# JeroendenBoef/GraphPOPE

Hardware: NVIDIA B200
Metric: anchor-BFS GTEPS (K*|E|/s), geodesic GraphPOPE embedding, Flickr-shape K=256 per GPU (higher is better)
Workload: dtype u64

## Files before the change

graphpope_b200/csrc/gp_api.cu:

```cuda
#include "gp_msbfs.cuh"

#include <algorithm>
#include <atomic>
#include <condition_variable>
#include <functional>
#include <mutex>
#if defined(__x86_64__) || defined(_M_X64)
#include <emmintrin.h>
#endif
#include <thread>
#include <vector>

#include <nvtx3/nvToolsExt.h>
#include <unistd.h>

bool gp_is_capturing();
bool gp_xcopy_tma_ok(const float *d_x, int64_t num_features, int64_t ld_x, const float *d_out, int64_t ld_out);
int gp_launch_xcopy_tma(const float *d_x, int64_t num_nodes, int64_t num_features, int64_t ld_x, float *d_out,
                        int64_t ld_out, cudaStream_t stream);
struct gp_exchange;
int gp_exchange_launch(gp_exchange *x, int parity, const float *d_x, int64_t f, int64_t ldx, float *d_out, int64_t ldo,
                       int64_t coff, cudaStream_t stream);
int gp_exchange_next_parity(gp_exchange *x);
static bool g_capturing_flag_for_count() { return gp_is_capturing(); }
void gp_count_launches(int n);

namespace {
thread_local char g_err[512] = "";
int g_sm_count = 0;
std::atomic<long long> g_launches{0};
}

static thread_local int g_capture_count = 0;
void gp_count_launch()
{
    if (g_capturing_flag_for_count()) ++g_capture_count;
    else g_launches.fetch_add(1, std::memory_order_relaxed);
}
void gp_count_launches(int n) { g_launches.fetch_add(n, std::memory_order_relaxed); }

extern "C" int64_t gp_launch_count(void) { return (int64_t)g_launches.load(); }

void gp_set_error(const char *fmt, ...)
{
    va_list ap;
    va_start(ap, fmt);
    vsnprintf(g_err, sizeof(g_err), fmt, ap);
    va_end(ap);
}

int gp_sm_count()
{
    if (g_sm_count == 0) {
        int dev = 0, sms = 0;
        if (cudaGetDevice(&dev) == cudaSuccess &&
            cudaDeviceGetAttribute(&sms, cudaDevAttrMultiProcessorCount, dev) == cudaSuccess && sms > 0)
            g_sm_count = sms;
        else
            return 148;
    }
    return g_sm_count;
}

const GpEnv &gp_env()
{
    static const GpEnv env = [] {
        auto geti = [](const char *name, int dflt) {
            const char *v = getenv(name);
            return v ? atoi(v) : dflt;
        };
        GpEnv e;
        e.use_graph = geti("GP_USE_GRAPH", 1);
        e.xcopy_overlap = geti("GP_XCOPY_OVERLAP", 0);
        e.xcopy_stages = geti("GP_XCOPY_STAGES", 4);
        e.xcopy_grid = geti("GP_XCOPY_GRID", 0);
        e.bfs_cfg = geti("GP_BFS_CFG", -1);
        e.bfs_no_map = getenv("GP_BFS_NO_MAP") != nullptr;
        e.bfs_mapg = getenv("GP_BFS_MAPG") != nullptr;
        e.bfs_trace = getenv("GP_BFS_TRACE") != nullptr;
        e.bfs_push = geti("GP_BFS_PUSH", 0);
        e.xchg_grid = geti("GP_XCHG_GRID", 0);
        e.xchg_debug = geti("GP_XCHG_DEBUG", 0);
        e.stage_events = geti("GP_STAGE_EVENTS", 0);
        e.pdl = geti("GP_PDL", 1);
        e.csr_trace = geti("GP_CSR_TRACE", 0);
        e.nvtx = geti("GP_NVTX", 1);
        return e;
    }();
    return env;
}

uint64_t gp_next_uid()
{
    static std::atomic<uint64_t> next{1};
    return next.fetch_add(1, std::memory_order_relaxed);
}

GpRange::GpRange(const char *name) : on(gp_env().nvtx != 0)
{
    if (on) nvtxRangePushA(name);
}
GpRange::~GpRange()
{
    if (on) nvtxRangePop();
}

extern "C" int gp_abi_version(void) { return GP_ABI_VERSION; }

extern "C" const char *gp_last_error(void) { return g_err; }

extern "C" const char *gp_status_string(int status)
{
    switch (status) {
        case GP_OK: return "ok";
        case GP_ERR_INVALID: return "invalid argument";
        case GP_ERR_CUDA: return "CUDA runtime error";
        case GP_ERR_OOM: return "out of memory";
        case GP_ERR_INDEX_RANGE: return "index outside [0, num_nodes)";
        case GP_ERR_LEVEL_OVERFLOW: return "hop distance does not fit uint16";
        case GP_ERR_UNSUPPORTED: return "unsupported size or option";
        case GP_ERR_NOT_CONVERGED: return "power iteration failed to converge";
        case GP_ERR_NO_DEVICE: return "no usable CUDA device";
        default: return "unknown status";
    }
}

extern "C" int gp_device_info(int32_t *sm_count, int32_t *cc_major, int32_t *cc_minor, char *name,
                              int64_t name_cap)
{
    int dev = 0, count = 0;
    if (cudaGetDeviceCount(&count) != cudaSuccess || count == 0) {
        cudaGetLastError();
        gp_set_error("no CUDA device is visible to this process");
        return GP_ERR_NO_DEVICE;
    }
    GP_CUDA_CHECK(cudaGetDevice(&dev));
    cudaDeviceProp prop;
    GP_CUDA_CHECK(cudaGetDeviceProperties(&prop, dev));
    if (sm_count) *sm_count = prop.multiProcessorCount;
    if (cc_major) *cc_major = prop.major;
    if (cc_minor) *cc_minor = prop.minor;
    if (name && name_cap > 0) {
        strncpy(name, prop.name, (size_t)name_cap - 1);
        name[name_cap - 1] = 0;
    }
    return GP_OK;
}

struct gp_ctx {
    std::mutex mutex;
    int64_t n = -1, e_cap = -1, k_cap = -1;
    uint32_t flags = 0;
    gp_csr *csr = nullptr;
    gp_msbfs *bfs = nullptr;
    int64_t *d_edges = nullptr;
    int64_t *d_anchors = nullptr;
    float *d_feat = nullptr;
    uint16_t *d_hops = nullptr;
    cudaStream_t stream = nullptr;
    float *h_ring[2] = {nullptr, nullptr};
    cudaEvent_t ring_ev[2] = {nullptr, nullptr};

    void release()
    {
        gp_msbfs_free(bfs);
        gp_csr_free(csr);
        cudaFree(d_edges);
        cudaFree(d_anchors);
        cudaFree(d_feat);
        cudaFree(d_hops);
        bfs = nullptr;
        csr = nullptr;
        d_edges = nullptr;
        d_anchors = nullptr;
        d_feat = nullptr;
        d_hops = nullptr;
        n = e_cap = k_cap = -1;
    }
};

typedef gp_ctx HostCtx;

namespace {

HostCtx &default_ctx()
{
    static HostCtx ctx;
    return ctx;
}

int ensure_ctx(HostCtx &c, int64_t n, int64_t e, int64_t k, uint32_t flags)
{
    if (c.stream == nullptr) {
        GP_TRY(gp_device_info(nullptr, nullptr, nullptr, nullptr, 0));
        GP_CUDA_CHECK(cudaStreamCreateWithFlags(&c.stream, cudaStreamNonBlocking));
    }
    if (c.n == n && c.flags == flags && e <= c.e_cap && k <= c.k_cap) return GP_OK;
    c.release();
    GP_TRY(gp_csr_create(n, e, flags, &c.csr));
    GP_TRY(gp_msbfs_create(c.csr, k, &c.bfs));
    GP_CUDA_CHECK(cudaMalloc(&c.d_edges, sizeof(int64_t) * (size_t)std::max<int64_t>(2 * e, 2)));
    GP_CUDA_CHECK(cudaMalloc(&c.d_anchors, sizeof(int64_t) * (size_t)std::max<int64_t>(k, 1)));
    GP_CUDA_CHECK(cudaMalloc(&c.d_feat, sizeof(float) * (size_t)std::max<int64_t>(n * k, 1)));
    GP_CUDA_CHECK(cudaMalloc(&c.d_hops, sizeof(uint16_t) * (size_t)std::max<int64_t>(n * k, 1)));
    c.n = n;
    c.e_cap = e;
    c.k_cap = k;
    c.flags = flags;
    return GP_OK;
}

class HostPool {
public:
    static HostPool &get()
    {
        static HostPool pool;
        return pool;
    }
    void parallel_rows(int64_t rows, int64_t chunk, const std::function<void(int64_t, int64_t)> &fn)
    {
        std::unique_lock<std::mutex> run_lock(run_mutex_, std::try_to_lock);
        if (getpid() != owner_pid_ || !run_lock.owns_lock()) {
            fn(0, rows);
            return;
        }
        {
            std::lock_guard<std::mutex> lk(m_);
            fn_ = &fn;
            rows_ = rows;
            chunk_ = chunk;
            next_.store(0);
            pending_ = (int)workers_.size();
            ++epoch_;
        }
        cv_.notify_all();
        work();
        std::unique_lock<std::mutex> lk(m_);
        done_cv_.wait(lk, [&] { return pending_ == 0; });
        fn_ = nullptr;
    }

private:
    HostPool() : owner_pid_(getpid())
    {
        int nt = (int)std::min<unsigned>(std::max(1u, std::thread::hardware_concurrency()), 16u) - 1;
        for (int t = 0; t < nt; ++t) workers_.emplace_back([this] { loop(); });
    }
    ~HostPool()
    {
        if (getpid() != owner_pid_) {
            for (auto &t : workers_) t.detach();
            return;
        }
        {
            std::lock_guard<std::mutex> lk(m_);
            stop_ = true;
        }
        cv_.notify_all();
        for (auto &t : workers_) t.join();
    }
    void work()
    {
        for (;;) {
            const int64_t r0 = next_.fetch_add(chunk_);
            if (r0 >= rows_) break;
            (*fn_)(r0, std::min(rows_, r0 + chunk_));
        }
    }
    void loop()
    {
        uint64_t seen = 0;
        for (;;) {
            {
                std::unique_lock<std::mutex> lk(m_);
                cv_.wait(lk, [&] { return stop_ || epoch_ != seen; });
                if (stop_) return;
                seen = epoch_;
            }
            work();
            {
                std::lock_guard<std::mutex> lk(m_);
                if (--pending_ == 0) done_cv_.notify_one();
            }
        }
    }
    const pid_t owner_pid_;
    std::vector<std::thread> workers_;
    std::mutex m_, run_mutex_;
    std::condition_variable cv_, done_cv_;
    const std::function<void(int64_t, int64_t)> *fn_ = nullptr;
    std::atomic<int64_t> next_{0};
    int64_t rows_ = 0, chunk_ = 1;
    int pending_ = 0;
    uint64_t epoch_ = 0;
    bool stop_ = false;
};

inline void copy_row_streaming(const float *src, float *dst, size_t n)
{
#if defined(__x86_64__) || defined(_M_X64)
    size_t i = 0;
    while (i < n && (reinterpret_cast<uintptr_t>(dst + i) & 15u)) {
        dst[i] = src[i];
        ++i;
    }
    for (; i + 16 <= n; i += 16) {
        const __m128i a = _mm_loadu_si128(reinterpret_cast<const __m128i *>(src + i));
        const __m128i b = _mm_loadu_si128(reinterpret_cast<const __m128i *>(src + i + 4));
        const __m128i c = _mm_loadu_si128(reinterpret_cast<const __m128i *>(src + i + 8));
        const __m128i d = _mm_loadu_si128(reinterpret_cast<const __m128i *>(src + i + 12));
        _mm_stream_si128(reinterpret_cast<__m128i *>(dst + i), a);
        _mm_stream_si128(reinterpret_cast<__m128i *>(dst + i + 4), b);
        _mm_stream_si128(reinterpret_cast<__m128i *>(dst + i + 8), c);
        _mm_stream_si128(reinterpret_cast<__m128i *>(dst + i + 12), d);
    }
    for (; i + 4 <= n; i += 4)
        _mm_stream_si128(reinterpret_cast<__m128i *>(dst + i), _mm_loadu_si128(reinterpret_cast<const __m128i *>(src + i)));
    for (; i < n; ++i) dst[i] = src[i];
#else
    memcpy(dst, src, n * sizeof(float));
#endif
}

void copy_rows_parallel(const float *src, int64_t ld_src, float *dst, int64_t ld_dst, int64_t rows,
                        int64_t cols)
{
    if (rows <= 0 || cols <= 0) return;
    auto work = [=](int64_t r0, int64_t r1) {
        for (int64_t r = r0; r < r1; ++r) copy_row_streaming(src + r * ld_src, dst + r * ld_dst, (size_t)cols);
#if defined(__x86_64__) || defined(_M_X64)
        _mm_sfence();
#endif
    };
    if (rows * cols < (1 << 20)) {
        work(0, rows);
        return;
    }
    HostPool::get().parallel_rows(rows, 512, work);
}

}

namespace {

struct PipeKey {
    uint64_t csr, bfs, xchg;
    const void *ei, *anchors, *x, *out;
    int64_t e, k, f, ldx, ldo, coff, parity;
    bool operator==(const PipeKey &o) const { return memcmp(this, &o, sizeof(PipeKey)) == 0; }
};

struct PipeEntry {
    PipeKey key;
    cudaGraphExec_t exec = nullptr;
    int seen = 0;
    int kernels = 0;
    bool has_events = false;
    uint64_t stamp = 0;
};

}

struct gp_pipe_cache {
    std::vector<PipeEntry> pipes;
    cudaStream_t capture_stream = nullptr;
    uint64_t clock = 0;
};

namespace {

thread_local bool g_capturing = false;

struct SideCopy {
    cudaStream_t stream = nullptr;
    cudaEvent_t fork = nullptr, join = nullptr;
};

SideCopy &side_copy_state()
{
    static thread_local SideCopy sc;
    return sc;
}

int run_pipeline_eager(gp_csr *csr, gp_msbfs *bfs, const int64_t *d_ei, int64_t e, const int64_t *d_anchors,
                       int64_t k, const float *d_x, int64_t f, int64_t ldx, float *d_out, int64_t ldo,
                       int64_t coff, cudaStream_t s, gp_exchange *xchg = nullptr, int parity = 0)
{
    const int overlap = gp_env().xcopy_overlap;
    const bool have_copy = d_out != nullptr && d_x != nullptr && f > 0 && csr->num_nodes > 0 && xchg == nullptr;
    const bool tma_copy = have_copy && overlap == 2 && gp_xcopy_tma_ok(d_x, f, ldx, d_out, ldo);
    const bool side_copy = have_copy && (overlap == 1 || tma_copy);
    SideCopy &sc = side_copy_state();
    if (side_copy) {
        if (sc.stream == nullptr) {
            GP_CUDA_CHECK(cudaStreamCreateWithFlags(&sc.stream, cudaStreamNonBlocking));
            GP_CUDA_CHECK(cudaEventCreateWithFlags(&sc.fork, cudaEventDisableTiming));
            GP_CUDA_CHECK(cudaEventCreateWithFlags(&sc.join, cudaEventDisableTiming));
        }
        GP_CUDA_CHECK(cudaEventRecord(sc.fork, s));
        GP_CUDA_CHECK(cudaStreamWaitEvent(sc.stream, sc.fork, 0));
        int crc = GP_OK;
        if (tma_copy) {
            crc = gp_launch_xcopy_tma(d_x, csr->num_nodes, f, ldx, d_out, ldo, sc.stream);
        } else if (cudaMemcpy2DAsync(d_out, (size_t)ldo * sizeof(float), d_x, (size_t)ldx * sizeof(float),
                                     (size_t)f * sizeof(float), (size_t)csr->num_nodes, cudaMemcpyDeviceToDevice,
                                     sc.stream) != cudaSuccess) {
            gp_set_error("cudaMemcpy2DAsync of x failed");
            crc = GP_ERR_CUDA;
        }
        GP_CUDA_CHECK(cudaEventRecord(sc.join, sc.stream));
        if (crc != GP_OK) {
            cudaStreamWaitEvent(s, sc.join, 0);
            return crc;
        }
    }
    const unsigned ev_flags = gp_is_capturing() ? cudaEventRecordExternal : cudaEventRecordDefault;
    const bool stage_events = gp_stage_events_on(bfs);
    if (stage_events) GP_CUDA_CHECK(cudaEventRecordWithFlags(bfs->ev_pipe0, s, ev_flags));
    int rc;
    {
        GpRange r("graphpope:csr_build");
        rc = gp_csr_build(csr, d_ei, e, s);
    }
    if (rc == GP_OK) {
        GpRange r("graphpope:msbfs");
        bfs->push_edges = d_ei;
        bfs->push_num_edges = e;
        rc = gp_msbfs_run(bfs, d_anchors, k, s);
        bfs->push_edges = nullptr;
    }
    if (side_copy) GP_CUDA_CHECK(cudaStreamWaitEvent(s, sc.join, 0));
    GP_TRY(rc);
    GpRange r(xchg != nullptr ? "graphpope:exchange_decode" : "graphpope:epilogue");
    if (xchg != nullptr) GP_TRY(gp_exchange_launch(xchg, parity, d_x, f, ldx, d_out, ldo, coff, s));
    else if (d_out != nullptr) GP_TRY(gp_msbfs_features(bfs, side_copy ? nullptr : d_x, f, ldx, d_out, ldo, coff, s));
    else GP_TRY(gp_msbfs_pack(bfs, (int32_t)coff, nullptr, nullptr, nullptr, nullptr, nullptr, s));
    if (stage_events) GP_CUDA_CHECK(cudaEventRecordWithFlags(bfs->ev_pipe1, s, ev_flags));
    bfs->pipe_timed = stage_events;
    return GP_OK;
}

}

bool gp_is_capturing() { return g_capturing; }

void gp_pipe_cache_free(gp_pipe_cache *pc)
{
    if (pc == nullptr) return;
    for (auto &e : pc->pipes)
        if (e.exec) cudaGraphExecDestroy(e.exec);
    if (pc->capture_stream) cudaStreamDestroy(pc->capture_stream);
    delete pc;
}

uint64_t gp_exchange_uid(const gp_exchange *x);

static int geodesic_run_impl(gp_csr_t *csr, gp_msbfs_t *bfs, const int64_t *d_edge_index, int64_t num_edges,
                             const int64_t *d_anchors, int64_t num_anchors, const float *d_x,
                             int64_t num_features, int64_t ld_x, float *d_out, int64_t ld_out,
                             int64_t col_offset, gp_stream_t stream_, gp_exchange *xchg, int parity)
{
    cudaStream_t stream = (cudaStream_t)stream_;
    GP_REQUIRE(csr != nullptr && bfs != nullptr, GP_ERR_INVALID, "gp_geodesic_run: NULL handle");
    if (!gp_env().use_graph || csr->num_nodes == 0 || num_anchors == 0)
        return run_pipeline_eager(csr, bfs, d_edge_index, num_edges, d_anchors, num_anchors, d_x, num_features, ld_x,
                                  d_out, ld_out, col_offset, stream, xchg, parity);
    if (bfs->pipe_cache == nullptr) bfs->pipe_cache = new (std::nothrow) gp_pipe_cache();
    GP_REQUIRE(bfs->pipe_cache != nullptr, GP_ERR_OOM, "gp_geodesic_run: host allocation failed");
    gp_pipe_cache &pc = *bfs->pipe_cache;
    PipeKey key;
    memset(&key, 0, sizeof(key));
    key.csr = csr->uid; key.bfs = bfs->uid; key.ei = d_edge_index; key.anchors = d_anchors; key.x = d_x; key.out = d_out;
    key.e = num_edges; key.k = num_anchors; key.f = num_features; key.ldx = ld_x; key.ldo = ld_out; key.coff = col_offset;
    key.xchg = xchg ? gp_exchange_uid(xchg) : 0; key.parity = parity;
    PipeEntry *ent = nullptr;
    for (auto &p : pc.pipes)
        if (p.key == key) ent = &p;
    if (ent == nullptr) {
        if (pc.pipes.size() >= 8) {
            size_t lru = 0;
            for (size_t i = 1; i < pc.pipes.size(); ++i)
                if (pc.pipes[i].stamp < pc.pipes[lru].stamp) lru = i;
            if (pc.pipes[lru].exec) cudaGraphExecDestroy(pc.pipes[lru].exec);
            pc.pipes.erase(pc.pipes.begin() + lru);
        }
        pc.pipes.emplace_back();
        ent = &pc.pipes.back();
        ent->key = key;
    }
    ent->stamp = ++pc.clock;
    ent->seen += 1;
    if (ent->exec == nullptr && ent->seen == 2) {
        if (pc.capture_stream == nullptr)
            GP_CUDA_CHECK(cudaStreamCreateWithFlags(&pc.capture_stream, cudaStreamNonBlocking));
        cudaGraph_t graph = nullptr;
        if (cudaStreamBeginCapture(pc.capture_stream, cudaStreamCaptureModeRelaxed) == cudaSuccess) {
            g_capturing = true;
            g_capture_count = 0;
            const int rc = run_pipeline_eager(csr, bfs, d_edge_index, num_edges, d_anchors, num_anchors, d_x,
                                              num_features, ld_x, d_out, ld_out, col_offset, pc.capture_stream, xchg,
                                              parity);
            g_capturing = false;
            ent->kernels = g_capture_count;
            ent->has_events = bfs->pipe_timed;
            const cudaError_t ce = cudaStreamEndCapture(pc.capture_stream, &graph);
            if (rc == GP_OK && ce == cudaSuccess && graph != nullptr) {
                if (cudaGraphInstantiate(&ent->exec, graph, 0) != cudaSuccess) ent->exec = nullptr;
            }
            if (graph) cudaGraphDestroy(graph);
        }
        cudaGetLastError();
        if (ent->exec == nullptr) ent->seen = 1 << 20;
    }
    if (ent->exec != nullptr) {
        csr->in_built = false;
        csr->num_input_edges = num_edges;
        csr->built = true;
        gp_msbfs_layout(bfs, num_anchors);
        bfs->ran = true;
        bfs->pipe_timed = bfs->kernel_timed = ent->has_events;
        gp_count_launches(ent->kernels);
        GpRange r("graphpope:pipeline_graph_replay");
        GP_CUDA_CHECK(cudaGraphLaunch(ent->exec, stream));
        return GP_OK;
    }
    return run_pipeline_eager(csr, bfs, d_edge_index, num_edges, d_anchors, num_anchors, d_x, num_features, ld_x,
                              d_out, ld_out, col_offset, stream, xchg, parity);
}

extern "C" int gp_geodesic_run(gp_csr_t *csr, gp_msbfs_t *bfs, const int64_t *d_edge_index, int64_t num_edges,
                               const int64_t *d_anchors, int64_t num_anchors, const float *d_x,
                               int64_t num_features, int64_t ld_x, float *d_out, int64_t ld_out,
                               int64_t col_offset, gp_stream_t stream_)
{
    return geodesic_run_impl(csr, bfs, d_edge_index, num_edges, d_anchors, num_anchors, d_x, num_features, ld_x, d_out,
                             ld_out, col_offset, stream_, nullptr, 0);
}

extern "C" int gp_geodesic_run_exchange(gp_csr_t *csr, gp_msbfs_t *bfs, gp_exchange_t *xchg, const int64_t *d_edge_index,
                                        int64_t num_edges, const int64_t *d_anchors, int64_t num_anchors,
                                        const float *d_x, int64_t num_features, int64_t ld_x, float *d_out,
                                        int64_t ld_out, int64_t col_offset, gp_stream_t stream_)
{
    GP_REQUIRE(xchg != nullptr && d_out != nullptr, GP_ERR_INVALID, "gp_geodesic_run_exchange: NULL argument");
    GP_REQUIRE(csr != nullptr && csr->num_nodes > 0 && num_anchors > 0, GP_ERR_INVALID,
               "gp_geodesic_run_exchange: empty graph or shard");
    return geodesic_run_impl(csr, bfs, d_edge_index, num_edges, d_anchors, num_anchors, d_x, num_features, ld_x, d_out,
                             ld_out, col_offset, stream_, xchg, gp_exchange_next_parity(xchg));
}

extern "C" int gp_concat_x(const float *d_x, int64_t num_nodes, int64_t num_features, int64_t ld_x, float *d_out,
                           int64_t ld_out, gp_stream_t stream)
{
    GP_REQUIRE(num_nodes >= 0 && num_features >= 0 && ld_x >= num_features && ld_out >= num_features, GP_ERR_INVALID,
               "gp_concat_x: inconsistent sizes");
    if (num_nodes == 0 || num_features == 0) return GP_OK;
    GP_REQUIRE(d_x != nullptr && d_out != nullptr, GP_ERR_INVALID, "gp_concat_x: NULL argument");
    if (gp_xcopy_tma_ok(d_x, num_features, ld_x, d_out, ld_out))
        return gp_launch_xcopy_tma(d_x, num_nodes, num_features, ld_x, d_out, ld_out, (cudaStream_t)stream);
    GP_CUDA_CHECK(cudaMemcpy2DAsync(d_out, (size_t)ld_out * sizeof(float), d_x, (size_t)ld_x * sizeof(float),
                                    (size_t)num_features * sizeof(float), (size_t)num_nodes,
                                    cudaMemcpyDeviceToDevice, (cudaStream_t)stream));
    return GP_OK;
}

extern "C" int gp_geodesic_run_packed(gp_csr_t *csr, gp_msbfs_t *bfs, const int64_t *d_edge_index, int64_t num_edges,
                                      const int64_t *d_anchors, int64_t num_anchors, int32_t slot, gp_stream_t stream)
{
    GP_REQUIRE(slot == 0 || slot == 1, GP_ERR_INVALID, "gp_geodesic_run_packed: slot must be 0 or 1");
    return gp_geodesic_run(csr, bfs, d_edge_index, num_edges, d_anchors, num_anchors, nullptr, 0, 0, nullptr, 0, slot,
                           stream);
}

extern "C" int gp_host_concat(const float *h_x, int64_t num_features, const float *h_block, int64_t block_cols,
                              int64_t num_nodes, float *h_out, int64_t ld_out)
{
    GP_REQUIRE(num_nodes >= 0 && num_features >= 0 && block_cols >= 0 && ld_out >= num_features + block_cols,
               GP_ERR_INVALID, "gp_host_concat: inconsistent sizes");
    GP_REQUIRE(h_out != nullptr || num_nodes == 0, GP_ERR_INVALID, "gp_host_concat: out is NULL");
    if (h_x != nullptr) copy_rows_parallel(h_x, num_features, h_out, ld_out, num_nodes, num_features);
    if (h_block != nullptr) copy_rows_parallel(h_block, block_cols, h_out + num_features, ld_out, num_nodes, block_cols);
    return GP_OK;
}

extern "C" int gp_block_to_host(const float *d_block, int64_t num_nodes, int64_t block_cols, float *h_out,
                                int64_t ld_out, int64_t col_offset, gp_stream_t stream_)
{
    GP_REQUIRE(num_nodes >= 0 && block_cols >= 0 && col_offset >= 0 && ld_out >= col_offset + block_cols, GP_ERR_INVALID,
               "gp_block_to_host: inconsistent sizes");
    if (num_nodes == 0 || block_cols == 0) return GP_OK;
    GP_REQUIRE(d_block != nullptr && h_out != nullptr, GP_ERR_INVALID, "gp_block_to_host: NULL argument");
    cudaPointerAttributes attr;
    const bool pinned = cudaPointerGetAttributes(&attr, h_out) == cudaSuccess && attr.type == cudaMemoryTypeHost;
    cudaGetLastError();
    GP_REQUIRE(pinned, GP_ERR_INVALID, "gp_block_to_host: h_out must be pinned host memory");
    GP_CUDA_CHECK(cudaMemcpy2DAsync(h_out + col_offset, sizeof(float) * (size_t)ld_out, d_block,
                                    sizeof(float) * (size_t)block_cols, sizeof(float) * (size_t)block_cols,
                                    (size_t)num_nodes, cudaMemcpyDeviceToHost, (cudaStream_t)stream_));
    return GP_OK;
}

extern "C" int gp_ctx_create(gp_ctx_t **out)
{
    GP_REQUIRE(out != nullptr, GP_ERR_INVALID, "gp_ctx_create: out is NULL");
    *out = new (std::nothrow) gp_ctx();
    GP_REQUIRE(*out != nullptr, GP_ERR_OOM, "gp_ctx_create: host allocation failed");
    return GP_OK;
}

extern "C" int gp_ctx_free(gp_ctx_t *ctx)
{
    if (ctx == nullptr) return GP_OK;
    ctx->release();
    for (int i = 0; i < 2; ++i) {
        if (ctx->h_ring[i]) cudaFreeHost(ctx->h_ring[i]);
        if (ctx->ring_ev[i]) cudaEventDestroy(ctx->ring_ev[i]);
    }
    if (ctx->stream) cudaStreamDestroy(ctx->stream);
    delete ctx;
    return GP_OK;
}

extern "C" int gp_geodesic_embed_host(const int64_t *h_edge_index, int64_t num_edges, int64_t num_nodes,
                                      uint32_t csr_flags, const int64_t *h_anchors, int64_t num_anchors,
                                      const float *h_x, int64_t num_features, float *h_out, int64_t ld_out,
                                      int64_t col_offset, uint16_t *h_hops, gp_msbfs_stats_t *stats)
{
    return gp_geodesic_embed_host_ctx(&default_ctx(), h_edge_index, num_edges, num_nodes, csr_flags, h_anchors,
                                      num_anchors, h_x, num_features, h_out, ld_out, col_offset, h_hops, stats);
}

extern "C" int gp_geodesic_embed_host_ctx(gp_ctx_t *ctx, const int64_t *h_edge_index, int64_t num_edges,
                                          int64_t num_nodes, uint32_t csr_flags, const int64_t *h_anchors,
                                          int64_t num_anchors, const float *h_x, int64_t num_features, float *h_out,
                                          int64_t ld_out, int64_t col_offset, uint16_t *h_hops, gp_msbfs_stats_t *stats)
{
    GP_REQUIRE(ctx != nullptr, GP_ERR_INVALID, "gp_geodesic_embed_host_ctx: ctx is NULL");
    GP_REQUIRE(num_edges >= 0 && num_nodes >= 0 && num_anchors >= 0 && num_features >= 0, GP_ERR_INVALID,
               "gp_geodesic_embed_host: negative size");
    GP_REQUIRE(num_edges == 0 || h_edge_index != nullptr, GP_ERR_INVALID, "edge_index is NULL");
    GP_REQUIRE(num_anchors == 0 || h_anchors != nullptr, GP_ERR_INVALID, "anchors is NULL");
    GP_REQUIRE(h_out != nullptr || num_nodes == 0 || (num_anchors == 0 && h_x == nullptr), GP_ERR_INVALID,
               "out is NULL");
    GP_REQUIRE(col_offset >= 0 && ld_out >= col_offset + num_anchors && (h_x == nullptr || col_offset >= num_features),
               GP_ERR_INVALID, "gp_geodesic_embed_host: inconsistent ld_out / col_offset");
    HostCtx &c = *ctx;
    std::lock_guard<std::mutex> lock(c.mutex);
    GP_TRY(ensure_ctx(c, num_nodes, num_edges, num_anchors, csr_flags));
    GpRange range("graphpope:embed_host");
    cudaStream_t s = c.stream;
    if (num_edges > 0)
        GP_CUDA_CHECK(cudaMemcpyAsync(c.d_edges, h_edge_index, sizeof(int64_t) * 2 * (size_t)num_edges,
                                      cudaMemcpyHostToDevice, s));
    if (num_anchors > 0)
        GP_CUDA_CHECK(cudaMemcpyAsync(c.d_anchors, h_anchors, sizeof(int64_t) * (size_t)num_anchors,
                                      cudaMemcpyHostToDevice, s));
    GP_TRY(gp_csr_build(c.csr, c.d_edges, num_edges, s));
    GP_TRY(gp_msbfs_run(c.bfs, c.d_anchors, num_anchors, s));
    if (num_nodes > 0 && num_anchors > 0) {
        GP_TRY(gp_msbfs_features(c.bfs, nullptr, 0, 0, c.d_feat, num_anchors, 0, s));
        if (h_hops) GP_TRY(gp_msbfs_hops_u16(c.bfs, c.d_hops, num_anchors, 0, s));
    }
    const bool have_block = num_nodes > 0 && num_anchors > 0;
    bool staged = false;
    if (have_block) {
        cudaPointerAttributes attr;
        const bool pinned = cudaPointerGetAttributes(&attr, h_out) == cudaSuccess && attr.type == cudaMemoryTypeHost;
        cudaGetLastError();
        if (pinned) {
            GP_CUDA_CHECK(cudaMemcpy2DAsync(h_out + col_offset, sizeof(float) * (size_t)ld_out, c.d_feat,
                                            sizeof(float) * (size_t)num_anchors, sizeof(float) * (size_t)num_anchors,
                                            (size_t)num_nodes, cudaMemcpyDeviceToHost, s));
        } else {
            staged = true;
        }
        if (h_hops)
            GP_CUDA_CHECK(cudaMemcpyAsync(h_hops, c.d_hops, sizeof(uint16_t) * (size_t)(num_nodes * num_anchors),
                                          cudaMemcpyDeviceToHost, s));
    }
    if (staged) {
        constexpr size_t RING_BYTES = 8u << 20;
        for (int i = 0; i < 2; ++i) {
            if (c.h_ring[i] == nullptr) GP_CUDA_CHECK(cudaMallocHost((void **)&c.h_ring[i], RING_BYTES));
            if (c.ring_ev[i] == nullptr) GP_CUDA_CHECK(cudaEventCreateWithFlags(&c.ring_ev[i], cudaEventDisableTiming));
        }
        const int64_t rows_per = std::max<int64_t>(1, (int64_t)(RING_BYTES / (sizeof(float) * (size_t)num_anchors)));
        const int64_t chunks = gp_ceil_div(num_nodes, rows_per);
        auto enqueue = [&](int64_t i) -> int {
            const int64_t r0 = i * rows_per, r1 = std::min(num_nodes, r0 + rows_per);
            GP_CUDA_CHECK(cudaMemcpyAsync(c.h_ring[i & 1], c.d_feat + r0 * num_anchors,
                                          sizeof(float) * (size_t)((r1 - r0) * num_anchors), cudaMemcpyDeviceToHost, s));
            GP_CUDA_CHECK(cudaEventRecord(c.ring_ev[i & 1], s));
            return GP_OK;
        };
        GP_REQUIRE((size_t)num_anchors * sizeof(float) <= RING_BYTES, GP_ERR_UNSUPPORTED,
                   "gp_geodesic_embed_host: more than %zu anchors need a pinned output buffer", RING_BYTES / sizeof(float));
        for (int64_t i = 0; i < std::min<int64_t>(2, chunks); ++i) GP_TRY(enqueue(i));
        if (h_x != nullptr) copy_rows_parallel(h_x, num_features, h_out, ld_out, num_nodes, num_features);
        for (int64_t i = 0; i < chunks; ++i) {
            const int64_t r0 = i * rows_per, r1 = std::min(num_nodes, r0 + rows_per);
            GP_CUDA_CHECK(cudaEventSynchronize(c.ring_ev[i & 1]));
            copy_rows_parallel(c.h_ring[i & 1], num_anchors, h_out + r0 * ld_out + col_offset, ld_out, r1 - r0, num_anchors);
            if (i + 2 < chunks) GP_TRY(enqueue(i + 2));
        }
    } else if (h_x != nullptr) {
        copy_rows_parallel(h_x, num_features, h_out, ld_out, num_nodes, num_features);
    }
    gp_msbfs_stats_t local;
    GP_TRY(gp_msbfs_stats(c.bfs, stats ? stats : &local, s));
    return GP_OK;
}
```

graphpope_b200/csrc/gp_common.cuh:

```cuda
#pragma once

#include <cuda_runtime.h>
#include <stdint.h>
#include <stdio.h>
#include <stdarg.h>
#include <string.h>

#include "../../include/graphpope_b200.h"

typedef unsigned long long u64;
typedef unsigned int u32;

void gp_set_error(const char *fmt, ...);

#define GP_CUDA_CHECK(expr)                                                              \
    do {                                                                                 \
        cudaError_t _e = (expr);                                                         \
        if (_e != cudaSuccess) {                                                         \
            gp_set_error("%s failed: %s (%s:%d)", #expr, cudaGetErrorString(_e),         \
                         __FILE__, __LINE__);                                            \
            return (_e == cudaErrorMemoryAllocation) ? GP_ERR_OOM : GP_ERR_CUDA;         \
        }                                                                                \
    } while (0)

#define GP_REQUIRE(cond, status, ...)                                                    \
    do {                                                                                 \
        if (!(cond)) {                                                                   \
            gp_set_error(__VA_ARGS__);                                                   \
            return (status);                                                             \
        }                                                                                \
    } while (0)

#define GP_TRY(expr)                                                                     \
    do {                                                                                 \
        int _s = (expr);                                                                 \
        if (_s != GP_OK) return _s;                                                      \
    } while (0)

static inline int64_t gp_ceil_div(int64_t a, int64_t b) { return (a + b - 1) / b; }

enum : int { GP_DEV_ERR_EDGE_RANGE = 1, GP_DEV_ERR_ANCHOR_RANGE = 2, GP_DEV_ERR_LEVEL_OVERFLOW = 4 };

int gp_sm_count();

struct GpEnv {
    int use_graph;
    int xcopy_overlap;
    int xcopy_stages;
    int xcopy_grid;
    int bfs_cfg;
    int bfs_no_map;
    int bfs_mapg;
    int bfs_trace;
    int bfs_push;
    int xchg_grid;
    int xchg_debug;
    int stage_events;
    int pdl;
    int csr_trace;
    int nvtx;
};
const GpEnv &gp_env();
uint64_t gp_next_uid();

struct GpRange {
    explicit GpRange(const char *name);
    ~GpRange();
    bool on;
};

void gp_count_launch();
bool gp_is_capturing();
#define GP_LAUNCH(kernel, grid, block, smem, stream, ...)                         \
    do {                                                                          \
        gp_count_launch();                                                        \
        kernel<<<(grid), (block), (smem), (stream)>>>(__VA_ARGS__);               \
    } while (0)

#ifdef __CUDACC__
template <typename... KArgs, typename... Args>
static inline cudaError_t gp_launch_pdl(void (*kernel)(KArgs...), dim3 grid, dim3 block, size_t smem, cudaStream_t stream,
                                        Args... args)
{
    cudaLaunchConfig_t cfg = {};
    cfg.gridDim = grid;
    cfg.blockDim = block;
    cfg.dynamicSmemBytes = smem;
    cfg.stream = stream;
    cudaLaunchAttribute attr[1];
    attr[0].id = cudaLaunchAttributeProgrammaticStreamSerialization;
    attr[0].val.programmaticStreamSerializationAllowed = 1;
    cfg.attrs = attr;
    cfg.numAttrs = gp_env().pdl ? 1 : 0;
    return cudaLaunchKernelEx(&cfg, kernel, KArgs(args)...);
}
#define GP_LAUNCH_PDL(kernel, grid, block, smem, stream, ...)                                     \
    do {                                                                                          \
        gp_count_launch();                                                                        \
        GP_CUDA_CHECK(gp_launch_pdl(kernel, dim3(grid), dim3(block), (smem), (stream), __VA_ARGS__)); \
    } while (0)
#endif

#ifdef __CUDACC__

__device__ __forceinline__ void gp_pdl_enter()
{
    asm volatile("griddepcontrol.launch_dependents;" ::: "memory");
    asm volatile("griddepcontrol.wait;" ::: "memory");
}

constexpr u32 FULL_MASK = 0xFFFFFFFFu;

__device__ __forceinline__ u32 lane_id() { return threadIdx.x & 31u; }

__device__ __forceinline__ u64 shfl_xor_u64(u64 v, int m)
{
    u32 lo = (u32)v, hi = (u32)(v >> 32);
    lo = __shfl_xor_sync(FULL_MASK, lo, m);
    hi = __shfl_xor_sync(FULL_MASK, hi, m);
    return ((u64)hi << 32) | lo;
}

__device__ __forceinline__ u64 warp_or_u64(u64 v)
{
    u32 lo = __reduce_or_sync(FULL_MASK, (u32)v);
    u32 hi = __reduce_or_sync(FULL_MASK, (u32)(v >> 32));
    return ((u64)hi << 32) | lo;
}

__device__ __forceinline__ u32 ld_acquire_u32(const u32 *p)
{
    u32 v;
    asm volatile("ld.acquire.gpu.global.u32 %0, [%1];" : "=r"(v) : "l"(p) : "memory");
    return v;
}

__device__ __forceinline__ u32 ld_relaxed_u32(const u32 *p)
{
    u32 v;
    asm volatile("ld.relaxed.gpu.global.u32 %0, [%1];" : "=r"(v) : "l"(p) : "memory");
    return v;
}

__device__ __forceinline__ void st_relaxed_u32(u32 *p, u32 v)
{
    asm volatile("st.relaxed.gpu.global.u32 [%0], %1;" ::"l"(p), "r"(v) : "memory");
}

__device__ __forceinline__ void red_release_add_u32(u32 *p, u32 v)
{
    asm volatile("red.release.gpu.global.add.u32 [%0], %1;" ::"l"(p), "r"(v) : "memory");
}

__device__ __forceinline__ void grid_barrier(u32 *counter, u32 &target, u32 nblocks)
{
    target += nblocks;
    __syncthreads();
    if (threadIdx.x == 0) {
        red_release_add_u32(counter, 1u);
        while (ld_relaxed_u32(counter) < target) {
        }
        (void)ld_acquire_u32(counter);
    }
    __syncthreads();
}

#endif
```

graphpope_b200/csrc/gp_csr.cu:

```cuda
#include "gp_internal.h"

#include <algorithm>
#include <new>

namespace {

constexpr int SCAN_THREADS = 256;
constexpr int SCAN_IPT = 4;
constexpr int SCAN_TILE = SCAN_THREADS * SCAN_IPT;
constexpr int ROW_CH = 9;
constexpr int BIG_THREADS = 256;
constexpr int BIG_SMEM_ELEMS = 8192;

int launch_blocks(int64_t work, int threads)
{
    int64_t b = gp_ceil_div(work > 0 ? work : 1, threads);
    const int64_t cap = (int64_t)gp_sm_count() * 32;
    return (int)(b < cap ? b : cap);
}

int row_blocks(int64_t rows)
{
    int64_t b = gp_ceil_div(rows > 0 ? rows : 1, 8);
    const int64_t cap = (int64_t)gp_sm_count() * 64;
    return (int)(b < cap ? b : cap);
}

__device__ __forceinline__ void load_edges4(const long long *__restrict__ ei, long long e, long long i0, int vec,
                                            long long (&s)[4], long long (&d)[4], int &cnt)
{
    cnt = (int)(e - i0 < 4 ? e - i0 : 4);
    if (vec && cnt == 4) {
        const longlong2 a = __ldcs(reinterpret_cast<const longlong2 *>(ei + i0));
        const longlong2 b = __ldcs(reinterpret_cast<const longlong2 *>(ei + i0) + 1);
        const longlong2 c = __ldcs(reinterpret_cast<const longlong2 *>(ei + e + i0));
        const longlong2 f = __ldcs(reinterpret_cast<const longlong2 *>(ei + e + i0) + 1);
        s[0] = a.x; s[1] = a.y; s[2] = b.x; s[3] = b.y;
        d[0] = c.x; d[1] = c.y; d[2] = f.x; d[3] = f.y;
    } else {
#pragma unroll
        for (int q = 0; q < 4; ++q) {
            s[q] = q < cnt ? ei[i0 + q] : 0;
            d[q] = q < cnt ? ei[e + i0 + q] : 0;
        }
    }
}

__global__ void __launch_bounds__(256)
count_edges_kernel(const long long *__restrict__ ei, long long e, long long n, int symmetrize, int vec,
                   int *__restrict__ cnt, int *meta)
{
    const long long stride = (long long)gridDim.x * blockDim.x * 4;
    bool bad = false;
    for (long long i0 = ((long long)blockIdx.x * blockDim.x + threadIdx.x) * 4; i0 < e; i0 += stride) {
        long long s[4], d[4];
        int c;
        load_edges4(ei, e, i0, vec, s, d, c);
#pragma unroll
        for (int q = 0; q < 4; ++q) {
            if (q >= c) break;
            if (s[q] < 0 || d[q] < 0 || s[q] >= n || d[q] >= n) {
                bad = true;
                continue;
            }
            atomicAdd(cnt + s[q], 1);
            if (symmetrize) atomicAdd(cnt + d[q], 1);
        }
    }
    if (__any_sync(FULL_MASK, bad) && lane_id() == 0) atomicOr(&meta[GP_META_ERROR], GP_DEV_ERR_EDGE_RANGE);
}

__global__ void __launch_bounds__(256)
scatter_edges_kernel(const long long *__restrict__ ei, long long e, long long n, int symmetrize, int vec,
                     int *__restrict__ cursor, int *__restrict__ raw_col)
{
    gp_pdl_enter();
    const long long stride = (long long)gridDim.x * blockDim.x * 4;
    for (long long i0 = ((long long)blockIdx.x * blockDim.x + threadIdx.x) * 4; i0 < e; i0 += stride) {
        long long s[4], d[4];
        int c, pos[4], pos2[4];
        load_edges4(ei, e, i0, vec, s, d, c);
        bool ok[4];
#pragma unroll
        for (int q = 0; q < 4; ++q) {
            ok[q] = q < c && !(s[q] < 0 || d[q] < 0 || s[q] >= n || d[q] >= n);
            pos[q] = ok[q] ? atomicAdd(cursor + s[q], 1) : 0;
            pos2[q] = (ok[q] && symmetrize) ? atomicAdd(cursor + d[q], 1) : 0;
        }
#pragma unroll
        for (int q = 0; q < 4; ++q) {
            if (ok[q]) {
                raw_col[pos[q]] = (int)d[q];
                if (symmetrize) raw_col[pos2[q]] = (int)s[q];
            }
        }
    }
}

__global__ void count_in_kernel(const int *__restrict__ row_start, const int *__restrict__ deg,
                                const int *__restrict__ col, long long n, int *__restrict__ cnt)
{
    const long long warps = ((long long)gridDim.x * blockDim.x) >> 5;
    const int lane = lane_id();
    for (long long u = ((long long)blockIdx.x * blockDim.x + threadIdx.x) >> 5; u < n; u += warps) {
        const int s = row_start[u], t = s + deg[u];
        for (int j = s + lane; j < t; j += 32) atomicAdd(cnt + col[j], 1);
    }
}

__global__ void scatter_in_kernel(const int *__restrict__ row_start, const int *__restrict__ deg,
                                  const int *__restrict__ col, long long n, int *__restrict__ cursor,
                                  int *__restrict__ col_in)
{
    const long long warps = ((long long)gridDim.x * blockDim.x) >> 5;
    const int lane = lane_id();
    for (long long u = ((long long)blockIdx.x * blockDim.x + threadIdx.x) >> 5; u < n; u += warps) {
        const int s = row_start[u], t = s + deg[u];
        for (int j = s + lane; j < t; j += 32) col_in[atomicAdd(cursor + col[j], 1)] = (int)u;
    }
}

template <int CHN>
struct ScanStatus {
    static constexpr int STRIDE = 1 + 2 * CHN;
};

__device__ __forceinline__ int ld_acquire_i32(const int *p)
{
    int v;
    asm volatile("ld.acquire.gpu.global.s32 %0, [%1];" : "=r"(v) : "l"(p) : "memory");
    return v;
}

__device__ __forceinline__ void st_release_i32(int *p, int v)
{
    asm volatile("st.release.gpu.global.s32 [%0], %1;" ::"l"(p), "r"(v) : "memory");
}

template <int CHN, class IO, int IPT = SCAN_IPT>
__global__ void __launch_bounds__(SCAN_THREADS) chained_scan_kernel(IO io, long long count, int *status, int *ticket)
{
    constexpr int STRIDE = ScanStatus<CHN>::STRIDE;
    constexpr int SCAN_IPT = IPT;
    constexpr int SCAN_TILE = SCAN_THREADS * SCAN_IPT;
    __shared__ int s_tile;
    __shared__ int s_warp[SCAN_THREADS / 32][CHN];
    __shared__ int s_prefix[CHN];
    const int tid = threadIdx.x, lane = tid & 31, warp = tid >> 5;
    gp_pdl_enter();
    if (tid == 0) s_tile = atomicAdd(ticket, 1);
    __syncthreads();
    const int tile = s_tile;
    const long long ntiles = (count + SCAN_TILE - 1) / SCAN_TILE;
    if (tile >= ntiles) return;

    const long long base = (long long)tile * SCAN_TILE + (long long)tid * SCAN_IPT;
    int v[SCAN_IPT][CHN], tsum[CHN];
#pragma unroll
    for (int c = 0; c < CHN; ++c) tsum[c] = 0;
#pragma unroll
    for (int k = 0; k < SCAN_IPT; ++k) {
#pragma unroll
        for (int c = 0; c < CHN; ++c) v[k][c] = 0;
        if (base + k < count) io.load(base + k, v[k]);
#pragma unroll
        for (int c = 0; c < CHN; ++c) tsum[c] += v[k][c];
    }
    int texcl[CHN];
#pragma unroll
    for (int c = 0; c < CHN; ++c) {
        int x = tsum[c];
#pragma unroll
        for (int o = 1; o < 32; o <<= 1) {
            const int y = __shfl_up_sync(FULL_MASK, x, o);
            if (lane >= o) x += y;
        }
        if (lane == 31) s_warp[warp][c] = x;
        texcl[c] = x - tsum[c];
    }
    __syncthreads();
    int agg[CHN];
#pragma unroll
    for (int c = 0; c < CHN; ++c) {
        int wbase = 0, tot = 0;
#pragma unroll
        for (int w = 0; w < SCAN_THREADS / 32; ++w) {
            const int t = s_warp[w][c];
            if (w < warp) wbase += t;
            tot += t;
        }
        texcl[c] += wbase;
        agg[c] = tot;
    }
    int *st = status + (size_t)tile * STRIDE;
    if (warp == 0) {
        if (tile > 0) {
            if (lane < CHN) {
                int mine = 0;
#pragma unroll
                for (int c = 0; c < CHN; ++c)
                    if (c == lane) mine = agg[c];
                st[1 + lane] = mine;
                __threadfence();
            }
            __syncwarp();
            if (lane == 0) st_release_i32(st, 1);
        }
        int run[CHN];
#pragma unroll
        for (int c = 0; c < CHN; ++c) run[c] = 0;
        for (int t = tile - 1; t >= 0; t -= 32) {
            const int idx = t - lane;
            const int *pt = status + (size_t)(idx >= 0 ? idx : 0) * STRIDE;
            int f = idx >= 0 ? ld_acquire_i32(pt) : 2;
            while (__any_sync(FULL_MASK, f == 0))
                if (f == 0) f = ld_acquire_i32(pt);
            const u32 inc_mask = __ballot_sync(FULL_MASK, f == 2);
            const int first = inc_mask ? __ffs(inc_mask) - 1 : 32;
#pragma unroll
            for (int c = 0; c < CHN; ++c) {
                int val = 0;
                if (idx >= 0 && lane <= first) val = pt[1 + (lane == first ? CHN : 0) + c];
                run[c] += __reduce_add_sync(FULL_MASK, val);
            }
            if (inc_mask) break;
        }
        if (lane < CHN) {
            int mine = 0, r = 0;
#pragma unroll
            for (int c = 0; c < CHN; ++c)
                if (c == lane) {
                    mine = agg[c];
                    r = run[c];
                }
            st[1 + CHN + lane] = r + mine;
            s_prefix[lane] = r;
            __threadfence();
        }
        __syncwarp();
        if (lane == 0) st_release_i32(st, 2);
    }
    __syncthreads();
    int excl[CHN];
#pragma unroll
    for (int c = 0; c < CHN; ++c) excl[c] = s_prefix[c] + texcl[c];
#pragma unroll
    for (int k = 0; k < SCAN_IPT; ++k) {
        if (base + k < count) io.store(base + k, excl, v[k]);
#pragma unroll
        for (int c = 0; c < CHN; ++c) excl[c] += v[k][c];
    }
    if (tile == ntiles - 1 && tid == 0) {
        int total[CHN];
#pragma unroll
        for (int c = 0; c < CHN; ++c) total[c] = s_prefix[c] + agg[c];
        io.finish(total);
    }
}

struct PtrScanIo {
    const int *cnt;
    int *ptr;
    int *cursor;
    long long n;
    __device__ void load(long long i, int (&v)[1]) const
    {
        if (i < n) v[0] = cnt[i];
    }
    __device__ void store(long long i, const int (&excl)[1], const int (&)[1]) const
    {
        ptr[i] = excl[0];
        if (i < n) cursor[i] = excl[0];
    }
    __device__ void finish(const int (&)[1]) const {}
};

struct PtrScanBuildIo {
    const int *cnt;
    int *ptr;
    int *cursor;
    long long n;
    int *biglist;
    int *medlist;
    int *meta;
    __device__ void load(long long i, int (&v)[1]) const
    {
        if (i < n) v[0] = cnt[i];
    }
    __device__ void store(long long i, const int (&excl)[1], const int (&v)[1]) const
    {
        ptr[i] = excl[0];
        if (i < n) {
            cursor[i] = excl[0];
            if (v[0] > 128) biglist[atomicAdd(&meta[GP_META_NUM_BIG_ROWS], 1)] = (int)i;
            else if (v[0] > 16) medlist[atomicAdd(&meta[GP_META_NUM_MED_ROWS], 1)] = (int)i;
        }
    }
    __device__ void finish(const int (&)[1]) const {}
};

__device__ __forceinline__ int degree_class(int d)
{
    return d > GP_CHUNK_EDGES ? 0 : d > 64 ? 1 : d > 32 ? 2 : d > 16 ? 3 : d > 8 ? 4 : d > 4 ? 5 : 6;
}

struct RowScanIo {
    const int *deg;
    const int *row_start;
    int4 *desc;
    int off[GP_NUM_CLASSES];
    int *meta;
    long long n;
    __device__ void load(long long i, int (&v)[ROW_CH]) const
    {
        const int d = deg[i];
        const int c = degree_class(d);
        v[0] = d;
#pragma unroll
        for (int k = 0; k < GP_NUM_CLASSES; ++k)
            if (k == c) v[1 + k] = c == 0 ? (d + GP_CHUNK_EDGES - 1) / GP_CHUNK_EDGES : 1;
        v[8] = c == 0 ? 1 : 0;
    }
    __device__ void store(long long i, const int (&excl)[ROW_CH], const int (&v)[ROW_CH]) const
    {
        const int d = v[0];
        const int c = degree_class(d);
        int r = 0, base = 0;
#pragma unroll
        for (int k = 0; k < GP_NUM_CLASSES; ++k)
            if (k == c) {
                r = excl[1 + k];
                base = off[k];
            }
        const int s = row_start[i];
        if (c != 0) {
            desc[base + r] = make_int4((int)i, s, d, -1);
        } else {
            const int nch = (d + GP_CHUNK_EDGES - 1) / GP_CHUNK_EDGES;
            for (int k = 0; k < nch; ++k) {
                const int cnt = min(GP_CHUNK_EDGES, d - k * GP_CHUNK_EDGES);
                desc[base + r + k] = make_int4((int)i, s + k * GP_CHUNK_EDGES, cnt | (nch << 8) | (k == 0 ? 1 << 30 : 0), excl[8]);
            }
        }
    }
    __device__ void finish(const int (&total)[ROW_CH]) const
    {
        meta[GP_META_NUM_EDGES] = total[0];
        meta[GP_META_NUM_HUB_ROWS] = total[8];
        int ent = 0, slot = 0;
        for (int c = 0; c < GP_NUM_CLASSES; ++c) {
            const int g = c <= 1 ? 32 : (32 >> (c - 1));
            meta[GP_META_ENT_BASE + c] = ent;
            meta[GP_META_SLOT_BASE + c] = slot;
            ent += total[1 + c];
            slot += (int)(((long long)total[1 + c] * g + GP_SLOT_ALIGN - 1) / GP_SLOT_ALIGN * GP_SLOT_ALIGN);
        }
        meta[GP_META_ENT_BASE + GP_NUM_CLASSES] = ent;
        meta[GP_META_SLOT_BASE + GP_NUM_CLASSES] = slot;
    }
};

__device__ __forceinline__ int warp_sort32(int v, int lane)
{
#pragma unroll
    for (int k = 2; k <= 32; k <<= 1) {
        {
            const int o = __shfl_xor_sync(FULL_MASK, v, k - 1);
            v = (lane & (k >> 1)) ? max(v, o) : min(v, o);
        }
#pragma unroll
        for (int j = k >> 2; j > 0; j >>= 1) {
            const int o = __shfl_xor_sync(FULL_MASK, v, j);
            v = (lane & j) ? max(v, o) : min(v, o);
        }
    }
    return v;
}

template <int E>
__device__ __forceinline__ void warp_sort_multi(int (&v)[E], int lane)
{
#pragma unroll
    for (int k = 2; k <= 32 * E; k <<= 1) {
        if (k <= 32) {
#pragma unroll
            for (int e = 0; e < E; ++e) {
                const int o = __shfl_xor_sync(FULL_MASK, v[e], k - 1);
                v[e] = (lane & (k >> 1)) ? max(v[e], o) : min(v[e], o);
            }
        } else {
            const int em = (k >> 5) - 1;
            int o[E];
#pragma unroll
            for (int e = 0; e < E; ++e) o[e] = __shfl_xor_sync(FULL_MASK, v[e ^ em], 31);
#pragma unroll
            for (int e = 0; e < E; ++e) v[e] = (e & (k >> 6)) ? max(v[e], o[e]) : min(v[e], o[e]);
        }
#pragma unroll
        for (int j = k >> 2; j > 0; j >>= 1) {
            if (j >= 32) {
                const int ej = j >> 5;
#pragma unroll
                for (int e = 0; e < E; ++e)
                    if (!(e & ej)) {
                        const int lo = min(v[e], v[e | ej]), hi = max(v[e], v[e | ej]);
                        v[e] = lo;
                        v[e | ej] = hi;
                    }
            } else {
#pragma unroll
                for (int e = 0; e < E; ++e) {
                    const int o = __shfl_xor_sync(FULL_MASK, v[e], j);
                    v[e] = (lane & j) ? max(v[e], o) : min(v[e], o);
                }
            }
        }
    }
}

template <int E>
__device__ __forceinline__ int warp_row_sort_unique(int *colbuf, int s, int len, int lane)
{
    int v[E];
#pragma unroll
    for (int e = 0; e < E; ++e) v[e] = e * 32 + lane < len ? colbuf[s + e * 32 + lane] : 0x7FFFFFFF;
    if constexpr (E == 1) v[0] = warp_sort32(v[0], lane);
    else warp_sort_multi<E>(v, lane);
    int base = 0;
#pragma unroll
    for (int e = 0; e < E; ++e) {
        int prev = __shfl_up_sync(FULL_MASK, v[e], 1);
        if (e > 0) {
            const int last = __shfl_sync(FULL_MASK, v[e - 1], 31);
            if (lane == 0) prev = last;
        }
        const bool head = e * 32 + lane < len && ((e == 0 && lane == 0) || v[e] != prev);
        const u32 heads = __ballot_sync(FULL_MASK, head);
        if (head) colbuf[s + base + __popc(heads & ((1u << lane) - 1u))] = v[e];
        base += __popc(heads);
    }
    return base;
}

__device__ __forceinline__ int thread_row_sort_unique(int *colbuf, int s, int len)
{
    int v[8];
#pragma unroll
    for (int i = 0; i < 8; ++i) v[i] = i < len ? colbuf[s + i] : 0x7FFFFFFF;
#define GP_CE(a, b)                              \
    {                                            \
        const int lo = min(v[a], v[b]);          \
        v[b] = max(v[a], v[b]);                  \
        v[a] = lo;                               \
    }
    GP_CE(0, 1) GP_CE(2, 3) GP_CE(4, 5) GP_CE(6, 7)
    GP_CE(0, 2) GP_CE(1, 3) GP_CE(4, 6) GP_CE(5, 7)
    GP_CE(1, 2) GP_CE(5, 6) GP_CE(0, 4) GP_CE(3, 7)
    GP_CE(1, 5) GP_CE(2, 6)
    GP_CE(1, 4) GP_CE(3, 6)
    GP_CE(2, 4) GP_CE(3, 5)
    GP_CE(3, 4)
#undef GP_CE
    int d = 0;
#pragma unroll
    for (int i = 0; i < 8; ++i) {
        if (i < len && (i == 0 || v[i] != v[i - 1])) {
            colbuf[s + d] = v[i];
            ++d;
        }
    }
    return d;
}

__device__ __forceinline__ int thread_row_sort_unique16(int *colbuf, int s, int len)
{
    int v[16];
#pragma unroll
    for (int i = 0; i < 16; ++i) v[i] = i < len ? colbuf[s + i] : 0x7FFFFFFF;
#define GP_CE(a, b)                              \
    {                                            \
        const int lo = min(v[a], v[b]);          \
        v[b] = max(v[a], v[b]);                  \
        v[a] = lo;                               \
    }
    GP_CE(0, 1) GP_CE(2, 3) GP_CE(0, 2) GP_CE(1, 3) GP_CE(1, 2) GP_CE(4, 5) GP_CE(6, 7) GP_CE(4, 6)
    GP_CE(5, 7) GP_CE(5, 6) GP_CE(0, 4) GP_CE(2, 6) GP_CE(2, 4) GP_CE(1, 5) GP_CE(3, 7) GP_CE(3, 5)
    GP_CE(1, 2) GP_CE(3, 4) GP_CE(5, 6) GP_CE(8, 9) GP_CE(10, 11) GP_CE(8, 10) GP_CE(9, 11)
    GP_CE(9, 10) GP_CE(12, 13) GP_CE(14, 15) GP_CE(12, 14) GP_CE(13, 15) GP_CE(13, 14) GP_CE(8, 12)
    GP_CE(10, 14) GP_CE(10, 12) GP_CE(9, 13) GP_CE(11, 15) GP_CE(11, 13) GP_CE(9, 10) GP_CE(11, 12)
    GP_CE(13, 14) GP_CE(0, 8) GP_CE(4, 12) GP_CE(4, 8) GP_CE(2, 10) GP_CE(6, 14) GP_CE(6, 10)
    GP_CE(2, 4) GP_CE(6, 8) GP_CE(10, 12) GP_CE(1, 9) GP_CE(5, 13) GP_CE(5, 9) GP_CE(3, 11)
    GP_CE(7, 15) GP_CE(7, 11) GP_CE(3, 5) GP_CE(7, 9) GP_CE(11, 13) GP_CE(1, 2) GP_CE(3, 4) GP_CE(5, 6)
    GP_CE(7, 8) GP_CE(9, 10) GP_CE(11, 12) GP_CE(13, 14)
#undef GP_CE
    int d = 0;
#pragma unroll
    for (int i = 0; i < 16; ++i) {
        if (i < len && (i == 0 || v[i] != v[i - 1])) {
            colbuf[s + d] = v[i];
            ++d;
        }
    }
    return d;
}

__global__ void __launch_bounds__(256)
rowsort_small_kernel(const int *__restrict__ ptr, const int *len_in, int *__restrict__ colbuf, long long n, int *deg,
                     int *__restrict__ biglist, int *meta, int max_word, int collect_big)
{
    const int lane = lane_id();
    const long long nblk = (n + 255) / 256;
    int mx = 0;
    gp_pdl_enter();
    for (long long blk = blockIdx.x; blk < nblk; blk += gridDim.x) {
        const long long r = blk * 256 + threadIdx.x;
        int s = 0, len = 0;
        if (r < n) {
            s = ptr[r];
            len = len_in[r];
        }
        if (len > 0 && len <= 8) {
            const int d = thread_row_sort_unique(colbuf, s, len);
            if (d != len) deg[r] = d;
            mx = max(mx, d);
        } else if (len > 8 && len <= 16) {
            const int d = thread_row_sort_unique16(colbuf, s, len);
            if (d != len) deg[r] = d;
            mx = max(mx, d);
        }
        u32 longer = collect_big ? __ballot_sync(FULL_MASK, len > 16) : 0u;
        while (longer) {
            const int src = __ffs(longer) - 1;
            longer &= longer - 1;
            const int rs = __shfl_sync(FULL_MASK, s, src), rlen = __shfl_sync(FULL_MASK, len, src);
            const long long rr = r - lane + src;
            if (rlen > 128) {
                if (collect_big && lane == 0) biglist[atomicAdd(&meta[GP_META_NUM_BIG_ROWS], 1)] = (int)rr;
                continue;
            }
            int d;
            if (rlen <= 32) d = warp_row_sort_unique<1>(colbuf, rs, rlen, lane);
            else if (rlen <= 64) d = warp_row_sort_unique<2>(colbuf, rs, rlen, lane);
            else d = warp_row_sort_unique<4>(colbuf, rs, rlen, lane);
            if (lane == 0 && d != rlen) deg[rr] = d;
            mx = max(mx, d);
        }
    }
    mx = __reduce_max_sync(FULL_MASK, mx);
    if (lane == 0 && mx > 0 && mx > *(volatile int *)&meta[max_word]) atomicMax(&meta[max_word], mx);
}

template <bool FLIP>
__device__ __forceinline__ void network_step(int *a, int len, int pairs, int sh, int tid, int nthreads)
{
    const int h = 1 << sh;
    for (int p0 = tid; p0 < pairs; p0 += 4 * nthreads) {
        int i[4], o[4], x[4], y[4];
#pragma unroll
        for (int q = 0; q < 4; ++q) {
            const int p = p0 + q * nthreads;
            const int blk = p >> sh, off = p & (h - 1);
            i[q] = (blk << (sh + 1)) + off;
            o[q] = FLIP ? (blk << (sh + 1)) + 2 * h - 1 - off : i[q] + h;
            if (p >= pairs) o[q] = len;
            if (o[q] < len) {
                x[q] = a[i[q]];
                y[q] = a[o[q]];
            }
        }
#pragma unroll
        for (int q = 0; q < 4; ++q)
            if (o[q] < len && x[q] > y[q]) {
                a[i[q]] = y[q];
                a[o[q]] = x[q];
            }
    }
}

__global__ void __launch_bounds__(BIG_THREADS)
rowsort_big_kernel(const int *__restrict__ ptr, const int *len_in, int *colbuf, int *deg,
                   const int *__restrict__ biglist, int *meta, int max_word, int bitmap_words,
                   const int *__restrict__ medlist)
{
    extern __shared__ __align__(16) int s_buf[];
    __shared__ int s_warp[BIG_THREADS / 32];
    __shared__ int s_carry;
    const int tid = threadIdx.x, lane = tid & 31, warp = tid >> 5;
    gp_pdl_enter();
    const int nbig = meta[GP_META_NUM_BIG_ROWS];
    for (int q = blockIdx.x; q < nbig; q += gridDim.x) {
        const int r = biglist[q];
        const int s = ptr[r], len = len_in[r];
        __syncthreads();
        if (bitmap_words > 0 && (long long)len * 32 >= bitmap_words) {
            u32 *bm = reinterpret_cast<u32 *>(s_buf);
            for (int i = tid; i < bitmap_words; i += BIG_THREADS) bm[i] = 0;
            __syncthreads();
            for (int i = tid; i < len; i += BIG_THREADS) {
                const int v = colbuf[s + i];
                atomicOr(&bm[v >> 5], 1u << (v & 31));
            }
            __syncthreads();
            const int wpt = (bitmap_words + BIG_THREADS - 1) / BIG_THREADS;
            const int w0 = tid * wpt, w1 = min(bitmap_words, w0 + wpt);
            int cnt = 0;
            for (int w = w0; w < w1; ++w) cnt += __popc(bm[w]);
            int x = cnt;
#pragma unroll
            for (int o = 1; o < 32; o <<= 1) {
                const int y = __shfl_up_sync(FULL_MASK, x, o);
                if (lane >= o) x += y;
            }
            if (lane == 31) s_warp[warp] = x;
            __syncthreads();
            int wbase = 0, tot = 0;
#pragma unroll
            for (int w = 0; w < BIG_THREADS / 32; ++w) {
                const int t = s_warp[w];
                if (w < warp) wbase += t;
                tot += t;
            }
            int pos = s + wbase + x - cnt;
            for (int w = w0; w < w1; ++w) {
                u32 bits = bm[w];
                while (bits) {
                    const int b = __ffs(bits) - 1;
                    bits &= bits - 1;
                    colbuf[pos++] = (w << 5) + b;
                }
            }
            if (tid == 0) {
                if (tot != len) deg[r] = tot;
                if (tot > *(volatile int *)&meta[max_word]) atomicMax(&meta[max_word], tot);
            }
            continue;
        }
        const bool in_smem = len <= BIG_SMEM_ELEMS;
        int *a = in_smem ? s_buf : colbuf + s;
        if (in_smem)
            for (int i = tid; i < len; i += BIG_THREADS) s_buf[i] = colbuf[s + i];
        __syncthreads();
        int lg = 1;
        while ((1 << lg) < len) ++lg;
        const int pairs = 1 << (lg - 1);
        for (int kb = 1; kb <= lg; ++kb) {
            network_step<true>(a, len, pairs, kb - 1, tid, BIG_THREADS);
            __syncthreads();
            for (int jb = kb - 2; jb >= 0; --jb) {
                network_step<false>(a, len, pairs, jb, tid, BIG_THREADS);
                __syncthreads();
            }
        }
        if (tid == 0) s_carry = 0;
        __syncthreads();
        for (int base = 0; base < len; base += BIG_THREADS) {
            const int i = base + tid;
            int v = 0;
            bool head = false;
            if (i < len) {
                v = a[i];
                head = i == 0 || a[i - 1] != v;
            }
            const u32 heads = __ballot_sync(FULL_MASK, head);
            if (lane == 0) s_warp[warp] = __popc(heads);
            __syncthreads();
            int wbase = 0, tot = 0;
#pragma unroll
            for (int w = 0; w < BIG_THREADS / 32; ++w) {
                const int t = s_warp[w];
                if (w < warp) wbase += t;
                tot += t;
            }
            const int carry = s_carry;
            if (head) colbuf[s + carry + wbase + __popc(heads & ((1u << lane) - 1u))] = v;
            __syncthreads();
            if (tid == 0) s_carry = carry + tot;
            __syncthreads();
        }
        if (tid == 0) {
            if (s_carry != len) deg[r] = s_carry;
            if (s_carry > *(volatile int *)&meta[max_word]) atomicMax(&meta[max_word], s_carry);
        }
    }
    if (medlist != nullptr) {
        const int nmed = meta[GP_META_NUM_MED_ROWS];
        const int busy = nbig < (int)gridDim.x ? nbig : 0;
        const int wpc = BIG_THREADS / 32;
        const int nw = ((int)gridDim.x - busy) * wpc;
        int mx = 0;
        if ((int)blockIdx.x >= busy) {
            for (int q = ((int)blockIdx.x - busy) * wpc + warp; q < nmed; q += nw) {
                const int r = medlist[q];
                const int rs = ptr[r], rlen = len_in[r];
                int d;
                if (rlen <= 32) d = warp_row_sort_unique<1>(colbuf, rs, rlen, lane);
                else if (rlen <= 64) d = warp_row_sort_unique<2>(colbuf, rs, rlen, lane);
                else d = warp_row_sort_unique<4>(colbuf, rs, rlen, lane);
                if (lane == 0 && d != rlen) deg[r] = d;
                mx = max(mx, d);
            }
        }
        if (lane == 0 && mx > 0 && mx > *(volatile int *)&meta[max_word]) atomicMax(&meta[max_word], mx);
    }
}

__global__ void compare_csr_kernel(const int *__restrict__ row_start, const int *__restrict__ deg,
                                   const int *__restrict__ col, const int *__restrict__ rowptr_in,
                                   const int *__restrict__ col_in, long long n, int *meta)
{
    const long long warps = ((long long)gridDim.x * blockDim.x) >> 5;
    const int lane = lane_id();
    bool diff = false;
    for (long long u = ((long long)blockIdx.x * blockDim.x + threadIdx.x) >> 5; u < n; u += warps) {
        const int s = row_start[u], d = deg[u], si = rowptr_in[u];
        if (rowptr_in[u + 1] - si != d) {
            diff = true;
            continue;
        }
        for (int j = lane; j < d; j += 32)
            if (col[s + j] != col_in[si + j]) diff = true;
    }
    if (__any_sync(FULL_MASK, diff) && lane == 0) atomicExch(&meta[GP_META_IS_SYMMETRIC], 0);
}

__global__ void gather_rows_kernel(const int *__restrict__ row_start, const int *__restrict__ deg,
                                   const int *__restrict__ col, const int *__restrict__ rowptr, long long n,
                                   int *__restrict__ out)
{
    const long long warps = ((long long)gridDim.x * blockDim.x) >> 5;
    const int lane = lane_id();
    for (long long u = ((long long)blockIdx.x * blockDim.x + threadIdx.x) >> 5; u < n; u += warps) {
        const int s = row_start[u], d = deg[u], t = rowptr[u];
        for (int j = lane; j < d; j += 32) out[t + j] = col[s + j];
    }
}

__global__ void set_meta_kernel(int *meta, int idx, int value) { meta[idx] = value; }

int scan_tiles(int64_t count) { return (int)gp_ceil_div(count > 0 ? count : 1, SCAN_TILE); }

int sort_rows(gp_csr *c, const int *ptr, int *len, int *colbuf, int max_word, bool reset_queue, cudaStream_t stream)
{
    const int64_t n = c->num_nodes;
    if (reset_queue) GP_LAUNCH(set_meta_kernel, 1, 1, 0, stream, c->meta, GP_META_NUM_BIG_ROWS, 0);
    GP_LAUNCH_PDL(rowsort_small_kernel, launch_blocks(n, 256), 256, 0, stream, ptr, (const int *)len, colbuf, (long long)n, len,
                  c->biglist, c->meta, max_word, 1);
    GP_LAUNCH_PDL(rowsort_big_kernel, gp_sm_count() * 4, BIG_THREADS, (size_t)c->big_smem_bytes, stream, ptr,
                  (const int *)len, colbuf, len, (const int *)c->biglist, c->meta, max_word, c->bitmap_words,
                  (const int *)nullptr);
    return GP_OK;
}

int sort_rows_forked(gp_csr *c, const int *ptr, int *len, int *colbuf, int max_word, cudaStream_t stream)
{
    const int64_t n = c->num_nodes;
    if (c->side == nullptr) {
        GP_CUDA_CHECK(cudaStreamCreateWithFlags(&c->side, cudaStreamNonBlocking));
        GP_CUDA_CHECK(cudaEventCreateWithFlags(&c->ev_fork, cudaEventDisableTiming));
        GP_CUDA_CHECK(cudaEventCreateWithFlags(&c->ev_join, cudaEventDisableTiming));
    }
    GP_CUDA_CHECK(cudaEventRecord(c->ev_fork, stream));
    GP_CUDA_CHECK(cudaStreamWaitEvent(c->side, c->ev_fork, 0));
    GP_LAUNCH(rowsort_big_kernel, gp_sm_count() * 4, BIG_THREADS, (size_t)c->big_smem_bytes, c->side, ptr, (const int *)len,
              colbuf, len, (const int *)c->biglist, c->meta, max_word, c->bitmap_words, (const int *)c->medlist);
    GP_CUDA_CHECK(cudaEventRecord(c->ev_join, c->side));
    GP_LAUNCH_PDL(rowsort_small_kernel, launch_blocks(n, 256), 256, 0, stream, ptr, (const int *)len, colbuf, (long long)n, len,
                  c->biglist, c->meta, max_word, 0);
    GP_CUDA_CHECK(cudaStreamWaitEvent(stream, c->ev_join, 0));
    return GP_OK;
}

}

extern "C" int gp_csr_create(int64_t num_nodes, int64_t edge_capacity, uint32_t flags, gp_csr_t **out)
{
    GP_REQUIRE(out != nullptr, GP_ERR_INVALID, "gp_csr_create: out is NULL");
    *out = nullptr;
    GP_REQUIRE(num_nodes >= 0 && edge_capacity >= 0, GP_ERR_INVALID, "gp_csr_create: negative size");
    GP_REQUIRE(num_nodes < (1ll << 31) - 1, GP_ERR_UNSUPPORTED, "gp_csr_create: num_nodes must fit int32");
    const int64_t kcap = edge_capacity * ((flags & GP_CSR_SYMMETRIZE) ? 2 : 1);
    GP_REQUIRE(kcap < (1ll << 30) - 1, GP_ERR_UNSUPPORTED,
               "gp_csr_create: %lld edge keys exceed the 2^30-1 limit of this build", (long long)kcap);
    gp_csr *c = new (std::nothrow) gp_csr();
    GP_REQUIRE(c != nullptr, GP_ERR_OOM, "gp_csr_create: host allocation failed");
    c->num_nodes = num_nodes;
    c->edge_capacity = edge_capacity;
    c->key_capacity = kcap;
    c->flags = flags;
    c->hub_capacity = kcap / (GP_CHUNK_EDGES + 1) + 1;
    {
        const int64_t min_deg[GP_NUM_CLASSES] = {0, 65, 33, 17, 9, 5, 0};
        int64_t off = 0;
        for (int k = 0; k < GP_NUM_CLASSES; ++k) {
            int64_t cap = k == 0 ? kcap / GP_CHUNK_EDGES + c->hub_capacity + 1
                                 : (min_deg[k] ? std::min<int64_t>(num_nodes, kcap / min_deg[k]) : num_nodes) + 1;
            c->desc_off[k] = (int)off;
            off += cap;
        }
        GP_REQUIRE(off < (1ll << 31), GP_ERR_UNSUPPORTED, "gp_csr_create: work list too large for this build");
        c->desc_off[GP_NUM_CLASSES] = (int)off;
        c->desc_capacity = off;
    }
    c->big_capacity = kcap / 129 + 1;
    const int64_t words = (num_nodes + 31) / 32;
    c->bitmap_words = words * 4 <= 96 * 1024 ? (int)words : 0;
    c->big_smem_bytes = BIG_SMEM_ELEMS * (int)sizeof(int);
    if (c->bitmap_words * 4 > c->big_smem_bytes) c->big_smem_bytes = (c->bitmap_words * 4 + 15) / 16 * 16;
    if (cudaFuncSetAttribute(rowsort_big_kernel, cudaFuncAttributeMaxDynamicSharedMemorySize, 96 * 1024) != cudaSuccess) {
        cudaGetLastError();
        c->bitmap_words = c->bitmap_words * 4 <= BIG_SMEM_ELEMS * (int)sizeof(int) ? c->bitmap_words : 0;
        c->big_smem_bytes = BIG_SMEM_ELEMS * (int)sizeof(int);
    }
    const size_t kc = (size_t)(kcap > 0 ? kcap : 1), nn = (size_t)num_nodes;
    int rc = GP_OK;
    auto alloc = [&](void **p, size_t bytes) {
        if (rc != GP_OK) return;
        cudaError_t e = cudaMalloc(p, bytes > 0 ? bytes : 16);
        if (e != cudaSuccess) {
            gp_set_error("gp_csr_create: cudaMalloc(%zu) failed: %s", bytes, cudaGetErrorString(e));
            rc = (e == cudaErrorMemoryAllocation) ? GP_ERR_OOM : GP_ERR_CUDA;
        }
    };
    alloc((void **)&c->row_start, (nn + 1) * sizeof(int));
    alloc((void **)&c->cursor, (nn + 1) * sizeof(int));
    alloc((void **)&c->col, kc * sizeof(int));
    alloc((void **)&c->biglist, (size_t)c->big_capacity * sizeof(int));
    c->med_capacity = kcap / 17 + 1;
    alloc((void **)&c->medlist, (size_t)c->med_capacity * sizeof(int));
    alloc((void **)&c->desc, (size_t)c->desc_capacity * sizeof(int4));
    c->scan_b_offset = (size_t)scan_tiles(num_nodes + 1) * ScanStatus<1>::STRIDE;
    c->scan_status_words = c->scan_b_offset + (size_t)scan_tiles(num_nodes + 1) * ScanStatus<ROW_CH>::STRIDE + 8;
    alloc((void **)&c->meta, (GP_META_WORDS + c->scan_status_words + nn + 1) * sizeof(int));
    c->scan_status = c->meta != nullptr ? c->meta + GP_META_WORDS : nullptr;
    c->deg = c->meta != nullptr ? c->scan_status + c->scan_status_words : nullptr;
    if (rc != GP_OK) {
        gp_csr_free(c);
        return rc;
    }
    *out = c;
    return GP_OK;
}

int gp_csr_scratch(gp_csr *c, int slot, size_t bytes, void **out)
{
    GP_REQUIRE(c != nullptr && out != nullptr && slot >= 0 && slot < 16, GP_ERR_INVALID, "gp_csr_scratch: bad argument");
    if (bytes == 0) bytes = 16;
    if (c->scratch_bytes[slot] < bytes) {
        if (c->scratch[slot]) cudaFree(c->scratch[slot]);
        c->scratch[slot] = nullptr;
        c->scratch_bytes[slot] = 0;
        GP_CUDA_CHECK(cudaMalloc(&c->scratch[slot], bytes));
        c->scratch_bytes[slot] = bytes;
    }
    *out = c->scratch[slot];
    return GP_OK;
}

extern "C" int gp_csr_free(gp_csr_t *c)
{
    if (!c) return GP_OK;
    for (int i = 0; i < 16; ++i) cudaFree(c->scratch[i]);
    for (int i = 0; i < 12; ++i)
        if (c->trace_ev[i]) cudaEventDestroy(c->trace_ev[i]);
    if (c->ev_fork) cudaEventDestroy(c->ev_fork);
    if (c->ev_join) cudaEventDestroy(c->ev_join);
    if (c->side) cudaStreamDestroy(c->side);
    cudaFree(c->row_start);
    cudaFree(c->cursor);
    cudaFree(c->col);
    cudaFree(c->rowptr_in);
    cudaFree(c->col_in);
    cudaFree(c->deg_in);
    cudaFree(c->biglist);
    cudaFree(c->medlist);
    cudaFree(c->desc);
    cudaFree(c->meta);
    delete c;
    return GP_OK;
}

extern "C" int gp_csr_build(gp_csr_t *c, const int64_t *d_edge_index, int64_t num_edges, gp_stream_t stream_)
{
    cudaStream_t stream = (cudaStream_t)stream_;
    GP_REQUIRE(c != nullptr, GP_ERR_INVALID, "gp_csr_build: csr is NULL");
    GP_REQUIRE(num_edges >= 0 && num_edges <= c->edge_capacity, GP_ERR_INVALID,
               "gp_csr_build: %lld edges exceed the capacity %lld given to gp_csr_create",
               (long long)num_edges, (long long)c->edge_capacity);
    GP_REQUIRE(num_edges == 0 || d_edge_index != nullptr, GP_ERR_INVALID, "gp_csr_build: edge_index is NULL");
    const int sym = (c->flags & GP_CSR_SYMMETRIZE) ? 1 : 0;
    const int64_t n = c->num_nodes;
    c->num_input_edges = num_edges;
    c->built = false;
    c->in_built = false;
    c->trace_n = 0;
    auto mark = [&]() {
        if (!gp_env().csr_trace || c->trace_n >= 12) return;
        if (c->trace_ev[c->trace_n] == nullptr) cudaEventCreate(&c->trace_ev[c->trace_n]);
        cudaEventRecordWithFlags(c->trace_ev[c->trace_n++], stream,
                                 gp_is_capturing() ? cudaEventRecordExternal : cudaEventRecordDefault);
    };
    mark();
    GP_CUDA_CHECK(cudaMemsetAsync(c->meta, 0, (GP_META_WORDS + c->scan_status_words + (size_t)n + 1) * sizeof(int), stream));
    if (n > 0) {
        const long long *ei = (const long long *)d_edge_index;
        const int vec = (reinterpret_cast<uintptr_t>(ei) & 15u) == 0 && num_edges % 2 == 0;
        int *ticket_a = c->scan_status + c->scan_status_words - 8, *ticket_b = ticket_a + 1;
        mark();
        if (num_edges > 0)
            GP_LAUNCH(count_edges_kernel, launch_blocks(gp_ceil_div(num_edges, 4), 256), 256, 0, stream, ei, num_edges, n, sym,
                      vec, c->deg, c->meta);
        mark();
        PtrScanBuildIo pio{c->deg, c->row_start, c->cursor, n, c->biglist, c->medlist, c->meta};
        gp_count_launch();
        GP_CUDA_CHECK(gp_launch_pdl(chained_scan_kernel<1, PtrScanBuildIo, SCAN_IPT>, dim3((unsigned)scan_tiles(n + 1)),
                                    dim3(SCAN_THREADS), 0, stream, pio, (long long)(n + 1), c->scan_status, ticket_a));
        mark();
        if (num_edges > 0)
            GP_LAUNCH_PDL(scatter_edges_kernel, launch_blocks(gp_ceil_div(num_edges, 4), 256), 256, 0, stream, ei,
                          (long long)num_edges, (long long)n, sym, vec, c->cursor, c->col);
        mark();
        GP_TRY(sort_rows_forked(c, c->row_start, c->deg, c->col, GP_META_MAX_DEGREE, stream));
        mark();
        RowScanIo rio;
        rio.deg = c->deg;
        rio.row_start = c->row_start;
        rio.desc = c->desc;
        for (int k = 0; k < GP_NUM_CLASSES; ++k) rio.off[k] = c->desc_off[k];
        rio.meta = c->meta;
        rio.n = n;
        gp_count_launch();
        GP_CUDA_CHECK(gp_launch_pdl(chained_scan_kernel<ROW_CH, RowScanIo, SCAN_IPT>, dim3((unsigned)scan_tiles(n)),
                                    dim3(SCAN_THREADS), 0, stream, rio, (long long)n, c->scan_status + c->scan_b_offset,
                                    ticket_b));
        mark();
        mark();
    }
    GP_CUDA_CHECK(cudaGetLastError());
    c->built = true;
    return GP_OK;
}

extern "C" int gp_csr_trace_ms(gp_csr_t *c, float *ms, int32_t cap, int32_t *num)
{
    GP_REQUIRE(c != nullptr && ms != nullptr && num != nullptr, GP_ERR_INVALID, "gp_csr_trace_ms: NULL argument");
    GP_REQUIRE(c->trace_n >= 2, GP_ERR_INVALID, "gp_csr_trace_ms: set GP_CSR_TRACE=1 and build first");
    GP_CUDA_CHECK(cudaEventSynchronize(c->trace_ev[c->trace_n - 1]));
    int k = 0;
    for (; k + 1 < c->trace_n && k < cap; ++k) GP_CUDA_CHECK(cudaEventElapsedTime(ms + k, c->trace_ev[k], c->trace_ev[k + 1]));
    *num = k;
    return GP_OK;
}

int gp_csr_ensure_in(gp_csr *c, cudaStream_t stream)
{
    GP_REQUIRE(c != nullptr && c->built, GP_ERR_INVALID, "in-edge CSR requested before gp_csr_build");
    if (c->in_built) return GP_OK;
    const int64_t n = c->num_nodes;
    if (c->rowptr_in == nullptr) {
        GP_REQUIRE(!gp_is_capturing(), GP_ERR_INVALID, "in-edge CSR cannot be allocated inside a graph capture");
        const size_t kc = (size_t)(c->key_capacity > 0 ? c->key_capacity : 1);
        GP_CUDA_CHECK(cudaMalloc((void **)&c->rowptr_in, (size_t)(n + 1) * sizeof(int)));
        GP_CUDA_CHECK(cudaMalloc((void **)&c->col_in, kc * sizeof(int)));
        GP_CUDA_CHECK(cudaMalloc((void **)&c->deg_in, (size_t)(n + 1) * sizeof(int)));
    }
    GP_LAUNCH(set_meta_kernel, 1, 1, 0, stream, c->meta, GP_META_IS_SYMMETRIC, 1);
    if (n > 0) {
        int *ticket = c->scan_status + c->scan_status_words - 8;
        GP_CUDA_CHECK(cudaMemsetAsync(c->deg_in, 0, (size_t)(n + 1) * sizeof(int), stream));
        GP_CUDA_CHECK(cudaMemsetAsync(c->scan_status, 0, c->scan_status_words * sizeof(int), stream));
        GP_LAUNCH(count_in_kernel, row_blocks(n), 256, 0, stream, c->row_start, c->deg, c->col, n, c->deg_in);
        PtrScanIo pio{c->deg_in, c->rowptr_in, c->cursor, n};
        gp_count_launch();
        chained_scan_kernel<1, PtrScanIo><<<scan_tiles(n + 1), SCAN_THREADS, 0, stream>>>(pio, n + 1, c->scan_status,
                                                                                        ticket);
        GP_LAUNCH(scatter_in_kernel, row_blocks(n), 256, 0, stream, c->row_start, c->deg, c->col, n, c->cursor,
                  c->col_in);
        GP_TRY(sort_rows(c, c->rowptr_in, c->deg_in, c->col_in, GP_META_SCRATCH, true, stream));
        GP_LAUNCH(compare_csr_kernel, row_blocks(n), 256, 0, stream, c->row_start, c->deg, c->col, c->rowptr_in,
                  c->col_in, n, c->meta);
    }
    GP_LAUNCH(set_meta_kernel, 1, 1, 0, stream, c->meta, GP_META_IN_BUILT, 1);
    GP_CUDA_CHECK(cudaGetLastError());
    c->in_built = true;
    return GP_OK;
}

extern "C" int gp_csr_info(gp_csr_t *c, gp_csr_info_t *info, gp_stream_t stream_)
{
    cudaStream_t stream = (cudaStream_t)stream_;
    GP_REQUIRE(c != nullptr && info != nullptr, GP_ERR_INVALID, "gp_csr_info: NULL argument");
    GP_REQUIRE(c->built, GP_ERR_INVALID, "gp_csr_info: gp_csr_build has not been called");
    GP_TRY(gp_csr_ensure_in(c, stream));
    int meta[GP_META_WORDS];
    GP_CUDA_CHECK(cudaMemcpyAsync(meta, c->meta, sizeof(meta), cudaMemcpyDeviceToHost, stream));
    GP_CUDA_CHECK(cudaStreamSynchronize(stream));
    info->num_nodes = c->num_nodes;
    info->num_input_edges = c->num_input_edges;
    info->num_edges = (u32)meta[GP_META_NUM_EDGES];
    info->max_out_degree = meta[GP_META_MAX_DEGREE];
    info->is_symmetric = meta[GP_META_IS_SYMMETRIC];
    info->reserved = 0;
    GP_REQUIRE(!(meta[GP_META_ERROR] & GP_DEV_ERR_EDGE_RANGE), GP_ERR_INDEX_RANGE,
               "edge_index holds an entry outside [0, %lld)", (long long)c->num_nodes);
    return GP_OK;
}

extern "C" int gp_csr_export(gp_csr_t *c, int which, int32_t *d_rowptr, int32_t *d_col, gp_stream_t stream_)
{
    cudaStream_t stream = (cudaStream_t)stream_;
    GP_REQUIRE(c != nullptr && d_rowptr != nullptr && d_col != nullptr, GP_ERR_INVALID,
               "gp_csr_export: NULL argument");
    GP_REQUIRE(c->built, GP_ERR_INVALID, "gp_csr_export: gp_csr_build has not been called");
    GP_REQUIRE(which == 0 || which == 1, GP_ERR_INVALID, "gp_csr_export: which must be 0 (out) or 1 (in)");
    const int64_t n = c->num_nodes;
    if (n == 0) {
        GP_CUDA_CHECK(cudaMemsetAsync(d_rowptr, 0, sizeof(int), stream));
        GP_CUDA_CHECK(cudaStreamSynchronize(stream));
        return GP_OK;
    }
    if (which == 1) {
        GP_TRY(gp_csr_ensure_in(c, stream));
        int m = 0;
        GP_CUDA_CHECK(cudaMemcpyAsync(&m, &c->meta[GP_META_NUM_EDGES], sizeof(int), cudaMemcpyDeviceToHost, stream));
        GP_CUDA_CHECK(cudaStreamSynchronize(stream));
        GP_CUDA_CHECK(cudaMemcpyAsync(d_rowptr, c->rowptr_in, (size_t)(n + 1) * sizeof(int), cudaMemcpyDeviceToDevice,
                                      stream));
        if (m > 0)
            GP_CUDA_CHECK(cudaMemcpyAsync(d_col, c->col_in, (size_t)(u32)m * sizeof(int), cudaMemcpyDeviceToDevice,
                                          stream));
    } else {
        int *ticket = c->scan_status + c->scan_status_words - 8;
        GP_CUDA_CHECK(cudaMemsetAsync(c->scan_status, 0, c->scan_status_words * sizeof(int), stream));
        PtrScanIo pio{c->deg, d_rowptr, c->cursor, n};
        gp_count_launch();
        chained_scan_kernel<1, PtrScanIo><<<scan_tiles(n + 1), SCAN_THREADS, 0, stream>>>(pio, n + 1, c->scan_status,
                                                                                        ticket);
        GP_LAUNCH(gather_rows_kernel, row_blocks(n), 256, 0, stream, c->row_start, c->deg, c->col, d_rowptr, n, d_col);
        GP_CUDA_CHECK(cudaGetLastError());
    }
    GP_CUDA_CHECK(cudaStreamSynchronize(stream));
    return GP_OK;
}
```

graphpope_b200/csrc/gp_internal.h:

```cpp
#pragma once

#include "gp_common.cuh"

constexpr int GP_SLOT_EDGES = 4;
constexpr int GP_CHUNK_EDGES = 32 * GP_SLOT_EDGES;
constexpr int GP_NUM_CLASSES = 7;
constexpr int GP_SLOT_ALIGN = 32;

static_assert(GP_CHUNK_EDGES == 128, "degree_class() in gp_csr.cu hard-codes the class thresholds");

enum : int {
    GP_META_NUM_EDGES = 0,
    GP_META_ERROR = 1,
    GP_META_NUM_BIG_ROWS = 2,
    GP_META_SCRATCH = 3,
    GP_META_MAX_DEGREE = 4,
    GP_META_IS_SYMMETRIC = 5,
    GP_META_IN_BUILT = 6,
    GP_META_NUM_HUB_ROWS = 7,
    GP_META_NUM_MED_ROWS = 8,
    GP_META_ENT_BASE = 16,
    GP_META_SLOT_BASE = 24,
    GP_META_WORDS = 32
};

struct gp_csr {
    uint64_t uid = gp_next_uid();
    int64_t num_nodes = 0;
    int64_t edge_capacity = 0;
    int64_t key_capacity = 0;
    int64_t num_input_edges = 0;
    uint32_t flags = 0;
    int64_t hub_capacity = 0;
    int64_t desc_capacity = 0;
    int desc_off[8] = {};
    int64_t big_capacity = 0;
    bool built = false;
    bool in_built = false;

    int *deg = nullptr;
    int *row_start = nullptr;
    int *col = nullptr;
    int *cursor = nullptr;
    int *rowptr_in = nullptr;
    int *col_in = nullptr;
    int *deg_in = nullptr;
    int *biglist = nullptr;
    int *medlist = nullptr;
    int64_t med_capacity = 0;
    int4 *desc = nullptr;
    int *meta = nullptr;
    int *scan_status = nullptr;
    size_t scan_status_words = 0;
    size_t scan_b_offset = 0;
    void *scratch[16] = {};
    size_t scratch_bytes[16] = {};
    cudaStream_t side = nullptr;
    cudaEvent_t ev_fork = nullptr, ev_join = nullptr;
    cudaEvent_t trace_ev[12] = {};
    int trace_n = 0;
    int bitmap_words = 0;
    int big_smem_bytes = 0;
};

int gp_csr_scratch(gp_csr *csr, int slot, size_t bytes, void **out);
int gp_csr_ensure_in(gp_csr *csr, cudaStream_t stream);
```

Baseline: 1031.

## Replace multi-kernel CSR build with a single cooperative bucketed build kernel

Replaces the CSR construction pipeline (count edges, chained scan, scatter, forked row sort, row-descriptor scan), which used PDL launches and a side stream, with one cooperative kernel. That kernel buckets edges into slabs in shared memory and uses grid barriers between phases. PDL helpers, the medium-row list and event-based tracing are removed, and tracing now uses device timestamps. This targets launch and inter-kernel overhead in graph preprocessing. It has little bearing on the anchor-BFS GTEPS metric unless the build is inside the timed region, and it adds grid-barrier and occupancy constraints.

```diff
diff --git a/graphpope_b200/csrc/gp_api.cu b/graphpope_b200/csrc/gp_api.cu
--- a/graphpope_b200/csrc/gp_api.cu
+++ b/graphpope_b200/csrc/gp_api.cu
@@ -82,7 +82,6 @@
         e.xchg_grid = geti("GP_XCHG_GRID", 0);
         e.xchg_debug = geti("GP_XCHG_DEBUG", 0);
         e.stage_events = geti("GP_STAGE_EVENTS", 0);
-        e.pdl = geti("GP_PDL", 1);
         e.csr_trace = geti("GP_CSR_TRACE", 0);
         e.nvtx = geti("GP_NVTX", 1);
         return e;
diff --git a/graphpope_b200/csrc/gp_common.cuh b/graphpope_b200/csrc/gp_common.cuh
--- a/graphpope_b200/csrc/gp_common.cuh
+++ b/graphpope_b200/csrc/gp_common.cuh
@@ -56,7 +56,6 @@
     int xchg_grid;
     int xchg_debug;
     int stage_events;
-    int pdl;
     int csr_trace;
     int nvtx;
 };
@@ -78,36 +77,6 @@
     } while (0)
 
 #ifdef __CUDACC__
-template <typename... KArgs, typename... Args>
-static inline cudaError_t gp_launch_pdl(void (*kernel)(KArgs...), dim3 grid, dim3 block, size_t smem, cudaStream_t stream,
-                                        Args... args)
-{
-    cudaLaunchConfig_t cfg = {};
-    cfg.gridDim = grid;
-    cfg.blockDim = block;
-    cfg.dynamicSmemBytes = smem;
-    cfg.stream = stream;
-    cudaLaunchAttribute attr[1];
-    attr[0].id = cudaLaunchAttributeProgrammaticStreamSerialization;
-    attr[0].val.programmaticStreamSerializationAllowed = 1;
-    cfg.attrs = attr;
-    cfg.numAttrs = gp_env().pdl ? 1 : 0;
-    return cudaLaunchKernelEx(&cfg, kernel, KArgs(args)...);
-}
-#define GP_LAUNCH_PDL(kernel, grid, block, smem, stream, ...)                                     \
-    do {                                                                                          \
-        gp_count_launch();                                                                        \
-        GP_CUDA_CHECK(gp_launch_pdl(kernel, dim3(grid), dim3(block), (smem), (stream), __VA_ARGS__)); \
-    } while (0)
-#endif
-
-#ifdef __CUDACC__
-
-__device__ __forceinline__ void gp_pdl_enter()
-{
-    asm volatile("griddepcontrol.launch_dependents;" ::: "memory");
-    asm volatile("griddepcontrol.wait;" ::: "memory");
-}
 
 constexpr u32 FULL_MASK = 0xFFFFFFFFu;
 
diff --git a/graphpope_b200/csrc/gp_csr.cu b/graphpope_b200/csrc/gp_csr.cu
--- a/graphpope_b200/csrc/gp_csr.cu
+++ b/graphpope_b200/csrc/gp_csr.cu
@@ -11,6 +11,13 @@
 constexpr int ROW_CH = 9;
 constexpr int BIG_THREADS = 256;
 constexpr int BIG_SMEM_ELEMS = 8192;
+
+constexpr int CB_THREADS = BIG_THREADS;
+constexpr int CB_STAGE = 12288;
+constexpr int CB_MAX_R = 2048;
+constexpr int CB_MAX_SLABS = 6144;
+constexpr int CB_SMEM_INTS = 3 * CB_MAX_R + CB_STAGE > 2 * CB_MAX_SLABS ? 3 * CB_MAX_R + CB_STAGE : 2 * CB_MAX_SLABS;
+constexpr int CB_CTL = 16;
 
 int launch_blocks(int64_t work, int threads)
 {
@@ -46,57 +53,6 @@
     }
 }
 
-__global__ void __launch_bounds__(256)
-count_edges_kernel(const long long *__restrict__ ei, long long e, long long n, int symmetrize, int vec,
-                   int *__restrict__ cnt, int *meta)
-{
-    const long long stride = (long long)gridDim.x * blockDim.x * 4;
-    bool bad = false;
-    for (long long i0 = ((long long)blockIdx.x * blockDim.x + threadIdx.x) * 4; i0 < e; i0 += stride) {
-        long long s[4], d[4];
-        int c;
-        load_edges4(ei, e, i0, vec, s, d, c);
-#pragma unroll
-        for (int q = 0; q < 4; ++q) {
-            if (q >= c) break;
-            if (s[q] < 0 || d[q] < 0 || s[q] >= n || d[q] >= n) {
-                bad = true;
-                continue;
-            }
-            atomicAdd(cnt + s[q], 1);
-            if (symmetrize) atomicAdd(cnt + d[q], 1);
-        }
-    }
-    if (__any_sync(FULL_MASK, bad) && lane_id() == 0) atomicOr(&meta[GP_META_ERROR], GP_DEV_ERR_EDGE_RANGE);
-}
-
-__global__ void __launch_bounds__(256)
-scatter_edges_kernel(const long long *__restrict__ ei, long long e, long long n, int symmetrize, int vec,
-                     int *__restrict__ cursor, int *__restrict__ raw_col)
-{
-    gp_pdl_enter();
-    const long long stride = (long long)gridDim.x * blockDim.x * 4;
-    for (long long i0 = ((long long)blockIdx.x * blockDim.x + threadIdx.x) * 4; i0 < e; i0 += stride) {
-        long long s[4], d[4];
-        int c, pos[4], pos2[4];
-        load_edges4(ei, e, i0, vec, s, d, c);
-        bool ok[4];
-#pragma unroll
-        for (int q = 0; q < 4; ++q) {
-            ok[q] = q < c && !(s[q] < 0 || d[q] < 0 || s[q] >= n || d[q] >= n);
-            pos[q] = ok[q] ? atomicAdd(cursor + s[q], 1) : 0;
-            pos2[q] = (ok[q] && symmetrize) ? atomicAdd(cursor + d[q], 1) : 0;
-        }
-#pragma unroll
-        for (int q = 0; q < 4; ++q) {
-            if (ok[q]) {
-                raw_col[pos[q]] = (int)d[q];
-                if (symmetrize) raw_col[pos2[q]] = (int)s[q];
-            }
-        }
-    }
-}
-
 __global__ void count_in_kernel(const int *__restrict__ row_start, const int *__restrict__ deg,
                                 const int *__restrict__ col, long long n, int *__restrict__ cnt)
 {
@@ -137,17 +93,97 @@
     asm volatile("st.release.gpu.global.s32 [%0], %1;" ::"l"(p), "r"(v) : "memory");
 }
 
-template <int CHN, class IO, int IPT = SCAN_IPT>
+template <int CHN>
+__device__ __forceinline__ void cta_scan(int (&x)[CHN], int (&tot)[CHN], int (*s_warp)[CHN])
+{
+    const int lane = threadIdx.x & 31, warp = threadIdx.x >> 5;
+#pragma unroll
+    for (int c = 0; c < CHN; ++c) {
+        int v = x[c];
+#pragma unroll
+        for (int o = 1; o < 32; o <<= 1) {
+            const int y = __shfl_up_sync(FULL_MASK, v, o);
+            if (lane >= o) v += y;
+        }
+        if (lane == 31) s_warp[warp][c] = v;
+        x[c] = v - x[c];
+    }
+    __syncthreads();
+#pragma unroll
+    for (int c = 0; c < CHN; ++c) {
+        int wbase = 0, t = 0;
+#pragma unroll
+        for (int w = 0; w < SCAN_THREADS / 32; ++w) {
+            const int u = s_warp[w][c];
+            if (w < warp) wbase += u;
+            t += u;
+        }
+        x[c] += wbase;
+        tot[c] = t;
+    }
+    __syncthreads();
+}
+
+template <int CHN>
+__device__ __forceinline__ void lookback_warp(int *status, int tile, const int (&agg)[CHN], int *s_prefix)
+{
+    constexpr int STRIDE = ScanStatus<CHN>::STRIDE;
+    const int lane = threadIdx.x & 31;
+    int *st = status + (size_t)tile * STRIDE;
+    if (tile > 0) {
+        if (lane < CHN) {
+            int mine = 0;
+#pragma unroll
+            for (int c = 0; c < CHN; ++c)
+                if (c == lane) mine = agg[c];
+            st[1 + lane] = mine;
+            __threadfence();
+        }
+        __syncwarp();
+        if (lane == 0) st_release_i32(st, 1);
+    }
+    int run[CHN];
+#pragma unroll
+    for (int c = 0; c < CHN; ++c) run[c] = 0;
+    for (int t = tile - 1; t >= 0; t -= 32) {
+        const int idx = t - lane;
+        const int *pt = status + (size_t)(idx >= 0 ? idx : 0) * STRIDE;
+        int f = idx >= 0 ? ld_acquire_i32(pt) : 2;
+        while (__any_sync(FULL_MASK, f == 0))
+            if (f == 0) f = ld_acquire_i32(pt);
+        const u32 inc_mask = __ballot_sync(FULL_MASK, f == 2);
+        const int first = inc_mask ? __ffs(inc_mask) - 1 : 32;
+#pragma unroll
+        for (int c = 0; c < CHN; ++c) {
+            int val = 0;
+            if (idx >= 0 && lane <= first) val = pt[1 + (lane == first ? CHN : 0) + c];
+            run[c] += __reduce_add_sync(FULL_MASK, val);
+        }
+        if (inc_mask) break;
+    }
+    if (lane < CHN) {
+        int mine = 0, r = 0;
+#pragma unroll
+        for (int c = 0; c < CHN; ++c)
+            if (c == lane) {
+                mine = agg[c];
+                r = run[c];
+            }
+        st[1 + CHN + lane] = r + mine;
+        s_prefix[lane] = r;
+        __threadfence();
+    }
+    __syncwarp();
+    if (lane == 0) st_release_i32(st, 2);
+}
+
+template <int CHN, class IO>
 __global__ void __launch_bounds__(SCAN_THREADS) chained_scan_kernel(IO io, long long count, int *status, int *ticket)
 {
-    constexpr int STRIDE = ScanStatus<CHN>::STRIDE;
-    constexpr int SCAN_IPT = IPT;
-    constexpr int SCAN_TILE = SCAN_THREADS * SCAN_IPT;
     __shared__ int s_tile;
     __shared__ int s_warp[SCAN_THREADS / 32][CHN];
     __shared__ int s_prefix[CHN];
-    const int tid = threadIdx.x, lane = tid & 31, warp = tid >> 5;
-    gp_pdl_enter();
+    const int tid = threadIdx.x;
     if (tid == 0) s_tile = atomicAdd(ticket, 1);
     __syncthreads();
     const int tile = s_tile;
@@ -155,95 +191,23 @@
     if (tile >= ntiles) return;
 
     const long long base = (long long)tile * SCAN_TILE + (long long)tid * SCAN_IPT;
-    int v[SCAN_IPT][CHN], tsum[CHN];
-#pragma unroll
-    for (int c = 0; c < CHN; ++c) tsum[c] = 0;
+    int v[SCAN_IPT][CHN], excl[CHN];
+#pragma unroll
+    for (int c = 0; c < CHN; ++c) excl[c] = 0;
 #pragma unroll
     for (int k = 0; k < SCAN_IPT; ++k) {
 #pragma unroll
         for (int c = 0; c < CHN; ++c) v[k][c] = 0;
         if (base + k < count) io.load(base + k, v[k]);
 #pragma unroll
-        for (int c = 0; c < CHN; ++c) tsum[c] += v[k][c];
-    }
-    int texcl[CHN];
-#pragma unroll
-    for (int c = 0; c < CHN; ++c) {
-        int x = tsum[c];
-#pragma unroll
-        for (int o = 1; o < 32; o <<= 1) {
-            const int y = __shfl_up_sync(FULL_MASK, x, o);
-            if (lane >= o) x += y;
-        }
-        if (lane == 31) s_warp[warp][c] = x;
-        texcl[c] = x - tsum[c];
-    }
-    __syncthreads();
+        for (int c = 0; c < CHN; ++c) excl[c] += v[k][c];
+    }
     int agg[CHN];
-#pragma unroll
-    for (int c = 0; c < CHN; ++c) {
-        int wbase = 0, tot = 0;
-#pragma unroll
-        for (int w = 0; w < SCAN_THREADS / 32; ++w) {
-            const int t = s_warp[w][c];
-            if (w < warp) wbase += t;
-            tot += t;
-        }
-        texcl[c] += wbase;
-        agg[c] = tot;
-    }
-    int *st = status + (size_t)tile * STRIDE;
-    if (warp == 0) {
-        if (tile > 0) {
-            if (lane < CHN) {
-                int mine = 0;
-#pragma unroll
-                for (int c = 0; c < CHN; ++c)
-                    if (c == lane) mine = agg[c];
-                st[1 + lane] = mine;
-                __threadfence();
-            }
-            __syncwarp();
-            if (lane == 0) st_release_i32(st, 1);
-        }
-        int run[CHN];
-#pragma unroll
-        for (int c = 0; c < CHN; ++c) run[c] = 0;
-        for (int t = tile - 1; t >= 0; t -= 32) {
-            const int idx = t - lane;
-            const int *pt = status + (size_t)(idx >= 0 ? idx : 0) * STRIDE;
-            int f = idx >= 0 ? ld_acquire_i32(pt) : 2;
-            while (__any_sync(FULL_MASK, f == 0))
-                if (f == 0) f = ld_acquire_i32(pt);
-            const u32 inc_mask = __ballot_sync(FULL_MASK, f == 2);
-            const int first = inc_mask ? __ffs(inc_mask) - 1 : 32;
-#pragma unroll
-            for (int c = 0; c < CHN; ++c) {
-                int val = 0;
-                if (idx >= 0 && lane <= first) val = pt[1 + (lane == first ? CHN : 0) + c];
-                run[c] += __reduce_add_sync(FULL_MASK, val);
-            }
-            if (inc_mask) break;
-        }
-        if (lane < CHN) {
-            int mine = 0, r = 0;
-#pragma unroll
-            for (int c = 0; c < CHN; ++c)
-                if (c == lane) {
-                    mine = agg[c];
-                    r = run[c];
-                }
-            st[1 + CHN + lane] = r + mine;
-            s_prefix[lane] = r;
-            __threadfence();
-        }
-        __syncwarp();
-        if (lane == 0) st_release_i32(st, 2);
-    }
-    __syncthreads();
-    int excl[CHN];
-#pragma unroll
-    for (int c = 0; c < CHN; ++c) excl[c] = s_prefix[c] + texcl[c];
+    cta_scan<CHN>(excl, agg, s_warp);
+    if (tid < 32) lookback_warp<CHN>(status, tile, agg, s_prefix);
+    __syncthreads();
+#pragma unroll
+    for (int c = 0; c < CHN; ++c) excl[c] += s_prefix[c];
 #pragma unroll
     for (int k = 0; k < SCAN_IPT; ++k) {
         if (base + k < count) io.store(base + k, excl, v[k]);
@@ -275,90 +239,58 @@
     __device__ void finish(const int (&)[1]) const {}
 };
 
-struct PtrScanBuildIo {
-    const int *cnt;
-    int *ptr;
-    int *cursor;
-    long long n;
-    int *biglist;
-    int *medlist;
-    int *meta;
-    __device__ void load(long long i, int (&v)[1]) const
-    {
-        if (i < n) v[0] = cnt[i];
-    }
-    __device__ void store(long long i, const int (&excl)[1], const int (&v)[1]) const
-    {
-        ptr[i] = excl[0];
-        if (i < n) {
-            cursor[i] = excl[0];
-            if (v[0] > 128) biglist[atomicAdd(&meta[GP_META_NUM_BIG_ROWS], 1)] = (int)i;
-            else if (v[0] > 16) medlist[atomicAdd(&meta[GP_META_NUM_MED_ROWS], 1)] = (int)i;
-        }
-    }
-    __device__ void finish(const int (&)[1]) const {}
-};
-
 __device__ __forceinline__ int degree_class(int d)
 {
     return d > GP_CHUNK_EDGES ? 0 : d > 64 ? 1 : d > 32 ? 2 : d > 16 ? 3 : d > 8 ? 4 : d > 4 ? 5 : 6;
 }
 
-struct RowScanIo {
-    const int *deg;
-    const int *row_start;
-    int4 *desc;
-    int off[GP_NUM_CLASSES];
-    int *meta;
-    long long n;
-    __device__ void load(long long i, int (&v)[ROW_CH]) const
-    {
-        const int d = deg[i];
-        const int c = degree_class(d);
-        v[0] = d;
-#pragma unroll
-        for (int k = 0; k < GP_NUM_CLASSES; ++k)
-            if (k == c) v[1 + k] = c == 0 ? (d + GP_CHUNK_EDGES - 1) / GP_CHUNK_EDGES : 1;
-        v[8] = c == 0 ? 1 : 0;
-    }
-    __device__ void store(long long i, const int (&excl)[ROW_CH], const int (&v)[ROW_CH]) const
-    {
-        const int d = v[0];
-        const int c = degree_class(d);
-        int r = 0, base = 0;
-#pragma unroll
-        for (int k = 0; k < GP_NUM_CLASSES; ++k)
-            if (k == c) {
-                r = excl[1 + k];
-                base = off[k];
-            }
-        const int s = row_start[i];
-        if (c != 0) {
-            desc[base + r] = make_int4((int)i, s, d, -1);
-        } else {
-            const int nch = (d + GP_CHUNK_EDGES - 1) / GP_CHUNK_EDGES;
-            for (int k = 0; k < nch; ++k) {
-                const int cnt = min(GP_CHUNK_EDGES, d - k * GP_CHUNK_EDGES);
-                desc[base + r + k] = make_int4((int)i, s + k * GP_CHUNK_EDGES, cnt | (nch << 8) | (k == 0 ? 1 << 30 : 0), excl[8]);
-            }
-        }
-    }
-    __device__ void finish(const int (&total)[ROW_CH]) const
-    {
-        meta[GP_META_NUM_EDGES] = total[0];
-        meta[GP_META_NUM_HUB_ROWS] = total[8];
-        int ent = 0, slot = 0;
-        for (int c = 0; c < GP_NUM_CLASSES; ++c) {
-            const int g = c <= 1 ? 32 : (32 >> (c - 1));
-            meta[GP_META_ENT_BASE + c] = ent;
-            meta[GP_META_SLOT_BASE + c] = slot;
-            ent += total[1 + c];
-            slot += (int)(((long long)total[1 + c] * g + GP_SLOT_ALIGN - 1) / GP_SLOT_ALIGN * GP_SLOT_ALIGN);
-        }
-        meta[GP_META_ENT_BASE + GP_NUM_CLASSES] = ent;
-        meta[GP_META_SLOT_BASE + GP_NUM_CLASSES] = slot;
-    }
-};
+__device__ __forceinline__ void row_channels(int d, int (&v)[ROW_CH])
+{
+    const int c = degree_class(d);
+    v[0] += d;
+#pragma unroll
+    for (int k = 0; k < GP_NUM_CLASSES; ++k)
+        if (k == c) v[1 + k] += c == 0 ? (d + GP_CHUNK_EDGES - 1) / GP_CHUNK_EDGES : 1;
+    v[8] += c == 0 ? 1 : 0;
+}
+
+__device__ __forceinline__ void store_desc(int4 *desc, const int (&off)[GP_NUM_CLASSES], int i, int s, int d,
+                                           const int (&excl)[ROW_CH])
+{
+    const int c = degree_class(d);
+    int r = 0, base = 0;
+#pragma unroll
+    for (int k = 0; k < GP_NUM_CLASSES; ++k)
+        if (k == c) {
+            r = excl[1 + k];
+            base = off[k];
+        }
+    if (c != 0) {
+        desc[base + r] = make_int4(i, s, d, -1);
+    } else {
+        const int nch = (d + GP_CHUNK_EDGES - 1) / GP_CHUNK_EDGES;
+        for (int k = 0; k < nch; ++k) {
+            const int cnt = min(GP_CHUNK_EDGES, d - k * GP_CHUNK_EDGES);
+            desc[base + r + k] = make_int4(i, s + k * GP_CHUNK_EDGES, cnt | (nch << 8) | (k == 0 ? 1 << 30 : 0), excl[8]);
+        }
+    }
+}
+
+__device__ __forceinline__ void write_meta(int *meta, const int (&total)[ROW_CH])
+{
+    meta[GP_META_NUM_EDGES] = total[0];
+    meta[GP_META_NUM_HUB_ROWS] = total[8];
+    int ent = 0, slot = 0;
+    for (int c = 0; c < GP_NUM_CLASSES; ++c) {
+        const int g = c <= 1 ? 32 : (32 >> (c - 1));
+        meta[GP_META_ENT_BASE + c] = ent;
+        meta[GP_META_SLOT_BASE + c] = slot;
+        ent += total[1 + c];
+        slot += (int)(((long long)total[1 + c] * g + GP_SLOT_ALIGN - 1) / GP_SLOT_ALIGN * GP_SLOT_ALIGN);
+    }
+    meta[GP_META_ENT_BASE + GP_NUM_CLASSES] = ent;
+    meta[GP_META_SLOT_BASE + GP_NUM_CLASSES] = slot;
+}
 
 __device__ __forceinline__ int warp_sort32(int v, int lane)
 {
@@ -504,14 +436,32 @@
     return d;
 }
 
+__device__ __noinline__ int warp_rows_sort_unique(int *colbuf, int s, int len, int lane)
+{
+    int d = len;
+    if (len > 0 && len <= 8) d = thread_row_sort_unique(colbuf, s, len);
+    else if (len > 8 && len <= 16) d = thread_row_sort_unique16(colbuf, s, len);
+    u32 longer = __ballot_sync(FULL_MASK, len > 16 && len <= 128);
+    while (longer) {
+        const int src = __ffs(longer) - 1;
+        longer &= longer - 1;
+        const int rs = __shfl_sync(FULL_MASK, s, src), rlen = __shfl_sync(FULL_MASK, len, src);
+        int w;
+        if (rlen <= 32) w = warp_row_sort_unique<1>(colbuf, rs, rlen, lane);
+        else if (rlen <= 64) w = warp_row_sort_unique<2>(colbuf, rs, rlen, lane);
+        else w = warp_row_sort_unique<4>(colbuf, rs, rlen, lane);
+        if (lane == src) d = w;
+    }
+    return d;
+}
+
 __global__ void __launch_bounds__(256)
 rowsort_small_kernel(const int *__restrict__ ptr, const int *len_in, int *__restrict__ colbuf, long long n, int *deg,
-                     int *__restrict__ biglist, int *meta, int max_word, int collect_big)
+                     int *__restrict__ biglist, int *meta, int max_word)
 {
     const int lane = lane_id();
     const long long nblk = (n + 255) / 256;
     int mx = 0;
-    gp_pdl_enter();
     for (long long blk = blockIdx.x; blk < nblk; blk += gridDim.x) {
         const long long r = blk * 256 + threadIdx.x;
         int s = 0, len = 0;
@@ -519,30 +469,11 @@
             s = ptr[r];
             len = len_in[r];
         }
-        if (len > 0 && len <= 8) {
-            const int d = thread_row_sort_unique(colbuf, s, len);
+        const int d = warp_rows_sort_unique(colbuf, s, len, lane);
+        if (len > 128) {
+            biglist[atomicAdd(&meta[GP_META_NUM_BIG_ROWS], 1)] = (int)r;
+        } else {
             if (d != len) deg[r] = d;
-            mx = max(mx, d);
-        } else if (len > 8 && len <= 16) {
-            const int d = thread_row_sort_unique16(colbuf, s, len);
-            if (d != len) deg[r] = d;
-            mx = max(mx, d);
-        }
-        u32 longer = collect_big ? __ballot_sync(FULL_MASK, len > 16) : 0u;
-        while (longer) {
-            const int src = __ffs(longer) - 1;
-            longer &= longer - 1;
-            const int rs = __shfl_sync(FULL_MASK, s, src), rlen = __shfl_sync(FULL_MASK, len, src);
-            const long long rr = r - lane + src;
-            if (rlen > 128) {
-                if (collect_big && lane == 0) biglist[atomicAdd(&meta[GP_META_NUM_BIG_ROWS], 1)] = (int)rr;
-                continue;
-            }
-            int d;
-            if (rlen <= 32) d = warp_row_sort_unique<1>(colbuf, rs, rlen, lane);
-            else if (rlen <= 64) d = warp_row_sort_unique<2>(colbuf, rs, rlen, lane);
-            else d = warp_row_sort_unique<4>(colbuf, rs, rlen, lane);
-            if (lane == 0 && d != rlen) deg[rr] = d;
             mx = max(mx, d);
         }
     }
@@ -577,131 +508,309 @@
     }
 }
 
+__device__ __noinline__ int cta_row_sort_unique(int *row, int len, int *buf, int cap, int *s_warp, int *s_carry)
+{
+    const int tid = threadIdx.x, lane = tid & 31, warp = tid >> 5;
+    int *a = row;
+    if (buf != row && len <= cap) {
+        a = buf;
+        for (int i = tid; i < len; i += BIG_THREADS) buf[i] = row[i];
+    }
+    __syncthreads();
+    int lg = 1;
+    while ((1 << lg) < len) ++lg;
+    const int pairs = 1 << (lg - 1);
+    for (int kb = 1; kb <= lg; ++kb) {
+        network_step<true>(a, len, pairs, kb - 1, tid, BIG_THREADS);
+        __syncthreads();
+        for (int jb = kb - 2; jb >= 0; --jb) {
+            network_step<false>(a, len, pairs, jb, tid, BIG_THREADS);
+            __syncthreads();
+        }
+    }
+    if (tid == 0) *s_carry = 0;
+    __syncthreads();
+    for (int base = 0; base < len; base += BIG_THREADS) {
+        const int i = base + tid;
+        int v = 0;
+        bool head = false;
+        if (i < len) {
+            v = a[i];
+            head = i == 0 || a[i - 1] != v;
+        }
+        const u32 heads = __ballot_sync(FULL_MASK, head);
+        if (lane == 0) s_warp[warp] = __popc(heads);
+        __syncthreads();
+        int wbase = 0, tot = 0;
+#pragma unroll
+        for (int w = 0; w < BIG_THREADS / 32; ++w) {
+            const int t = s_warp[w];
+            if (w < warp) wbase += t;
+            tot += t;
+        }
+        const int carry = *s_carry;
+        if (head) row[carry + wbase + __popc(heads & ((1u << lane) - 1u))] = v;
+        __syncthreads();
+        if (tid == 0) *s_carry = carry + tot;
+        __syncthreads();
+    }
+    return *s_carry;
+}
+
+__device__ __noinline__ int cta_bitmap_sort_unique(int *row, int len, u32 *bm, int words, int *s_warp)
+{
+    const int tid = threadIdx.x, lane = tid & 31, warp = tid >> 5;
+    for (int i = tid; i < words; i += BIG_THREADS) bm[i] = 0;
+    __syncthreads();
+    for (int i = tid; i < len; i += BIG_THREADS) {
+        const int v = row[i];
+        atomicOr(&bm[v >> 5], 1u << (v & 31));
+    }
+    __syncthreads();
+    const int wpt = (words + BIG_THREADS - 1) / BIG_THREADS;
+    const int w0 = tid * wpt, w1 = min(words, w0 + wpt);
+    int cnt = 0;
+    for (int w = w0; w < w1; ++w) cnt += __popc(bm[w]);
+    int x = cnt;
+#pragma unroll
+    for (int o = 1; o < 32; o <<= 1) {
+        const int y = __shfl_up_sync(FULL_MASK, x, o);
+        if (lane >= o) x += y;
+    }
+    if (lane == 31) s_warp[warp] = x;
+    __syncthreads();
+    int wbase = 0, tot = 0;
+#pragma unroll
+    for (int w = 0; w < BIG_THREADS / 32; ++w) {
+        const int t = s_warp[w];
+        if (w < warp) wbase += t;
+        tot += t;
+    }
+    int pos = wbase + x - cnt;
+    for (int w = w0; w < w1; ++w) {
+        u32 bits = bm[w];
+        while (bits) {
+            const int b = __ffs(bits) - 1;
+            bits &= bits - 1;
+            row[pos++] = (w << 5) + b;
+        }
+    }
+    __syncthreads();
+    return tot;
+}
+
 __global__ void __launch_bounds__(BIG_THREADS)
 rowsort_big_kernel(const int *__restrict__ ptr, const int *len_in, int *colbuf, int *deg,
-                   const int *__restrict__ biglist, int *meta, int max_word, int bitmap_words,
-                   const int *__restrict__ medlist)
+                   const int *__restrict__ biglist, int *meta, int max_word, int bitmap_words)
 {
     extern __shared__ __align__(16) int s_buf[];
     __shared__ int s_warp[BIG_THREADS / 32];
     __shared__ int s_carry;
     const int tid = threadIdx.x, lane = tid & 31, warp = tid >> 5;
-    gp_pdl_enter();
     const int nbig = meta[GP_META_NUM_BIG_ROWS];
     for (int q = blockIdx.x; q < nbig; q += gridDim.x) {
         const int r = biglist[q];
         const int s = ptr[r], len = len_in[r];
         __syncthreads();
-        if (bitmap_words > 0 && (long long)len * 32 >= bitmap_words) {
-            u32 *bm = reinterpret_cast<u32 *>(s_buf);
-            for (int i = tid; i < bitmap_words; i += BIG_THREADS) bm[i] = 0;
-            __syncthreads();
-            for (int i = tid; i < len; i += BIG_THREADS) {
-                const int v = colbuf[s + i];
-                atomicOr(&bm[v >> 5], 1u << (v & 31));
+        const int d = bitmap_words > 0 && (long long)len * 32 >= bitmap_words
+                          ? cta_bitmap_sort_unique(colbuf + s, len, reinterpret_cast<u32 *>(s_buf), bitmap_words, s_warp)
+                          : cta_row_sort_unique(colbuf + s, len, s_buf, BIG_SMEM_ELEMS, s_warp, &s_carry);
+        if (tid == 0) {
+            if (d != len) deg[r] = d;
+            if (d > *(volatile int *)&meta[max_word]) atomicMax(&meta[max_word], d);
+        }
+    }
+}
+
+struct CsrBuildParams {
+    const long long *ei;
+    long long e, n;
+    int sym, vec;
+    int lg;
+    int bitmap_words;
+    int slabs;
+    long long chunk;
+    u32 *bar;
+    unsigned long long *stamp;
+    int *slab_cnt, *slab_cur;
+    int *slab_off;
+    int *status;
+    int *bkt_col;
+    unsigned short *bkt_row;
+    int *row_start, *deg, *col;
+    int *biglist;
+    int4 *desc;
+    int desc_off[GP_NUM_CLASSES];
+    int *meta;
+};
+
+__device__ __forceinline__ void stamp_max(unsigned long long *w, bool invert)
+{
+    unsigned long long t;
+    asm volatile("mov.u64 %0, %%globaltimer;" : "=l"(t));
+    atomicMax(w, invert ? ~t : t);
+}
+
+template <class F>
+__device__ __forceinline__ bool for_chunk_edges(const CsrBuildParams &p, F f)
+{
+    const long long beg = (long long)blockIdx.x * p.chunk, end = min(p.e, beg + p.chunk);
+    bool bad = false;
+    for (long long i0 = beg + (long long)threadIdx.x * 4; i0 < end; i0 += CB_THREADS * 4) {
+        long long s[4], d[4];
+        int c;
+        load_edges4(p.ei, p.e, i0, p.vec, s, d, c);
+        int s32[4], d32[4];
+        u32 ok = 0;
+#pragma unroll
+        for (int q = 0; q < 4; ++q) {
+            const bool in = q < c && s[q] >= 0 && d[q] >= 0 && s[q] < p.n && d[q] < p.n;
+            bad |= q < c && !in;
+            ok |= in ? 1u << q : 0u;
+            s32[q] = (int)s[q];
+            d32[q] = (int)d[q];
+        }
+#pragma unroll
+        for (int q = 0; q < 4; ++q) {
+            if (!(ok >> q & 1u)) continue;
+            f(s32[q] >> p.lg, d32[q], s32[q] & ((1 << p.lg) - 1));
+            if (p.sym) f(d32[q] >> p.lg, s32[q], d32[q] & ((1 << p.lg) - 1));
+        }
+    }
+    return bad;
+}
+
+__global__ void __launch_bounds__(CB_THREADS, 2)
+csr_build_kernel(const CsrBuildParams p)
+{
+    extern __shared__ __align__(16) int s_dyn[];
+    __shared__ int s_warp[SCAN_THREADS / 32][ROW_CH];
+    __shared__ int s_prefix[ROW_CH];
+    __shared__ int s_carry;
+    const int tid = threadIdx.x, lane = tid & 31, warp = tid >> 5;
+    const int S = p.slabs, R = 1 << p.lg;
+    u32 target = 0;
+    if (p.stamp != nullptr && tid == 0) stamp_max(p.stamp + 0, true);
+
+    int *s_hist = s_dyn, *s_base = s_dyn + S;
+    for (int j = tid; j < S; j += CB_THREADS) s_hist[j] = 0;
+    __syncthreads();
+    const bool bad = for_chunk_edges(p, [s_hist](int slab, int, int) { atomicAdd(&s_hist[slab], 1); });
+    if (__any_sync(FULL_MASK, bad) && lane == 0) atomicOr(&p.meta[GP_META_ERROR], GP_DEV_ERR_EDGE_RANGE);
+    __syncthreads();
+    for (int j = tid; j < S; j += CB_THREADS)
+        if (s_hist[j] != 0) atomicAdd(&p.slab_cnt[j], s_hist[j]);
+    if (p.stamp != nullptr && tid == 0) stamp_max(p.stamp + 1, false);
+    grid_barrier(p.bar, target, gridDim.x);
+
+    {
+        const int per = (S + CB_THREADS - 1) / CB_THREADS, j0 = tid * per, j1 = min(S, j0 + per);
+        int x[1] = {0}, tot[1];
+        for (int j = j0; j < j1; ++j) x[0] += __ldcg(p.slab_cnt + j);
+        cta_scan<1>(x, tot, reinterpret_cast<int(*)[1]>(&s_warp[0][0]));
+        for (int j = j0; j < j1; ++j) {
+            const int c = __ldcg(p.slab_cnt + j);
+            if (blockIdx.x == 0) p.slab_off[j] = x[0];
+            s_base[j] = x[0] + (s_hist[j] != 0 ? atomicAdd(&p.slab_cur[j], s_hist[j]) : 0);
+            x[0] += c;
+        }
+    }
+    __syncthreads();
+    for_chunk_edges(p, [s_base, bkt_col = p.bkt_col, bkt_row = p.bkt_row](int slab, int dst, int row) {
+        const int pos = atomicAdd(&s_base[slab], 1);
+        bkt_col[pos] = dst;
+        bkt_row[pos] = (unsigned short)row;
+    });
+    if (p.stamp != nullptr && tid == 0) stamp_max(p.stamp + 2, false);
+    grid_barrier(p.bar, target, gridDim.x);
+
+    int *s_len = s_dyn, *s_pos = s_dyn + R, *s_cur = s_dyn + 2 * R, *s_stage = s_dyn + 3 * R;
+    const int rpt = (R + CB_THREADS - 1) / CB_THREADS;
+    int mx = 0;
+    for (int slab = blockIdx.x; slab < S; slab += gridDim.x) {
+        const int off = __ldcg(p.slab_off + slab), cnt = __ldcg(p.slab_cnt + slab);
+        const int r0 = slab << p.lg, nr = (int)min((long long)R, p.n - r0);
+        for (int j = tid; j < R; j += CB_THREADS) s_len[j] = 0;
+        __syncthreads();
+        for (int i = tid; i < cnt; i += CB_THREADS) atomicAdd(&s_len[__ldcg(p.bkt_row + off + i)], 1);
+        __syncthreads();
+        const int j0 = tid * rpt, j1 = min(nr, j0 + rpt);
+        {
+            int x[1] = {0}, tot[1];
+            for (int j = j0; j < j1; ++j) x[0] += s_len[j];
+            cta_scan<1>(x, tot, reinterpret_cast<int(*)[1]>(&s_warp[0][0]));
+            for (int j = j0; j < j1; ++j) {
+                s_pos[j] = s_cur[j] = x[0];
+                p.row_start[r0 + j] = off + x[0];
+                x[0] += s_len[j];
             }
-            __syncthreads();
-            const int wpt = (bitmap_words + BIG_THREADS - 1) / BIG_THREADS;
-            const int w0 = tid * wpt, w1 = min(bitmap_words, w0 + wpt);
-            int cnt = 0;
-            for (int w = w0; w < w1; ++w) cnt += __popc(bm[w]);
-            int x = cnt;
-#pragma unroll
-            for (int o = 1; o < 32; o <<= 1) {
-                const int y = __shfl_up_sync(FULL_MASK, x, o);
-                if (lane >= o) x += y;
-            }
-            if (lane == 31) s_warp[warp] = x;
-            __syncthreads();
-            int wbase = 0, tot = 0;
-#pragma unroll
-            for (int w = 0; w < BIG_THREADS / 32; ++w) {
-                const int t = s_warp[w];
-                if (w < warp) wbase += t;
-                tot += t;
-            }
-            int pos = s + wbase + x - cnt;
-            for (int w = w0; w < w1; ++w) {
-                u32 bits = bm[w];
-                while (bits) {
-                    const int b = __ffs(bits) - 1;
-                    bits &= bits - 1;
-                    colbuf[pos++] = (w << 5) + b;
-                }
-            }
-            if (tid == 0) {
-                if (tot != len) deg[r] = tot;
-                if (tot > *(volatile int *)&meta[max_word]) atomicMax(&meta[max_word], tot);
-            }
-            continue;
-        }
-        const bool in_smem = len <= BIG_SMEM_ELEMS;
-        int *a = in_smem ? s_buf : colbuf + s;
-        if (in_smem)
-            for (int i = tid; i < len; i += BIG_THREADS) s_buf[i] = colbuf[s + i];
-        __syncthreads();
-        int lg = 1;
-        while ((1 << lg) < len) ++lg;
-        const int pairs = 1 << (lg - 1);
-        for (int kb = 1; kb <= lg; ++kb) {
-            network_step<true>(a, len, pairs, kb - 1, tid, BIG_THREADS);
-            __syncthreads();
-            for (int jb = kb - 2; jb >= 0; --jb) {
-                network_step<false>(a, len, pairs, jb, tid, BIG_THREADS);
-                __syncthreads();
-            }
-        }
-        if (tid == 0) s_carry = 0;
-        __syncthreads();
-        for (int base = 0; base < len; base += BIG_THREADS) {
-            const int i = base + tid;
-            int v = 0;
-            bool head = false;
-            if (i < len) {
-                v = a[i];
-                head = i == 0 || a[i - 1] != v;
-            }
-            const u32 heads = __ballot_sync(FULL_MASK, head);
-            if (lane == 0) s_warp[warp] = __popc(heads);
-            __syncthreads();
-            int wbase = 0, tot = 0;
-#pragma unroll
-            for (int w = 0; w < BIG_THREADS / 32; ++w) {
-                const int t = s_warp[w];
-                if (w < warp) wbase += t;
-                tot += t;
-            }
-            const int carry = s_carry;
-            if (head) colbuf[s + carry + wbase + __popc(heads & ((1u << lane) - 1u))] = v;
-            __syncthreads();
-            if (tid == 0) s_carry = carry + tot;
-            __syncthreads();
-        }
-        if (tid == 0) {
-            if (s_carry != len) deg[r] = s_carry;
-            if (s_carry > *(volatile int *)&meta[max_word]) atomicMax(&meta[max_word], s_carry);
-        }
-    }
-    if (medlist != nullptr) {
-        const int nmed = meta[GP_META_NUM_MED_ROWS];
-        const int busy = nbig < (int)gridDim.x ? nbig : 0;
-        const int wpc = BIG_THREADS / 32;
-        const int nw = ((int)gridDim.x - busy) * wpc;
-        int mx = 0;
-        if ((int)blockIdx.x >= busy) {
-            for (int q = ((int)blockIdx.x - busy) * wpc + warp; q < nmed; q += nw) {
-                const int r = medlist[q];
-                const int rs = ptr[r], rlen = len_in[r];
-                int d;
-                if (rlen <= 32) d = warp_row_sort_unique<1>(colbuf, rs, rlen, lane);
-                else if (rlen <= 64) d = warp_row_sort_unique<2>(colbuf, rs, rlen, lane);
-                else d = warp_row_sort_unique<4>(colbuf, rs, rlen, lane);
-                if (lane == 0 && d != rlen) deg[r] = d;
-                mx = max(mx, d);
-            }
-        }
-        if (lane == 0 && mx > 0 && mx > *(volatile int *)&meta[max_word]) atomicMax(&meta[max_word], mx);
-    }
+        }
+        if (slab == S - 1 && tid == 0) p.row_start[p.n] = off + cnt;
+        __syncthreads();
+        int *a = cnt <= CB_STAGE ? s_stage : p.col + off;
+        for (int i = tid; i < cnt; i += CB_THREADS) {
+            const int v = __ldcg(p.bkt_col + off + i);
+            a[atomicAdd(&s_cur[__ldcg(p.bkt_row + off + i)], 1)] = v;
+        }
+        __syncthreads();
+        for (int j = warp * 32 + lane; j - lane < nr; j += CB_THREADS) {
+            const int len = j < nr ? s_len[j] : 0;
+            const int d = warp_rows_sort_unique(a, j < nr ? s_pos[j] : 0, len, lane);
+            if (j < nr) p.deg[r0 + j] = d;
+            if (len > 128) p.biglist[atomicAdd(&p.meta[GP_META_NUM_BIG_ROWS], 1)] = r0 + j;
+            else mx = max(mx, d);
+        }
+        __syncthreads();
+        if (a == s_stage)
+            for (int i = tid; i < cnt; i += CB_THREADS) p.col[off + i] = s_stage[i];
+        __syncthreads();
+    }
+    if (p.stamp != nullptr && tid == 0) stamp_max(p.stamp + 3, false);
+    grid_barrier(p.bar, target, gridDim.x);
+
+    const int nbig = __ldcg(p.meta + GP_META_NUM_BIG_ROWS);
+    for (int q = blockIdx.x; q < nbig; q += gridDim.x) {
+        const int r = __ldcg(p.biglist + q);
+        const int len = __ldcg(p.deg + r);
+        int *row = p.col + __ldcg(p.row_start + r);
+        const int d = p.bitmap_words > 0
+                          ? cta_bitmap_sort_unique(row, len, reinterpret_cast<u32 *>(s_dyn), p.bitmap_words, &s_warp[0][0])
+                          : cta_row_sort_unique(row, len, s_dyn, CB_SMEM_INTS, &s_warp[0][0], &s_carry);
+        if (tid == 0) p.deg[r] = d;
+        mx = max(mx, d);
+        __syncthreads();
+    }
+    mx = __reduce_max_sync(FULL_MASK, mx);
+    if (lane == 0 && mx > 0) atomicMax(&p.meta[GP_META_MAX_DEGREE], mx);
+    if (p.stamp != nullptr && tid == 0) stamp_max(p.stamp + 4, false);
+    grid_barrier(p.bar, target, gridDim.x);
+
+    for (int slab = blockIdx.x; slab < S; slab += gridDim.x) {
+        const int r0 = slab << p.lg, nr = (int)min((long long)R, p.n - r0);
+        const int j0 = tid * rpt, j1 = min(nr, j0 + rpt);
+        int v[ROW_CH], agg[ROW_CH];
+#pragma unroll
+        for (int c = 0; c < ROW_CH; ++c) v[c] = 0;
+        for (int j = j0; j < j1; ++j) row_channels(__ldcg(p.deg + r0 + j), v);
+        cta_scan<ROW_CH>(v, agg, s_warp);
+        if (warp == 0) lookback_warp<ROW_CH>(p.status, slab, agg, s_prefix);
+        __syncthreads();
+#pragma unroll
+        for (int c = 0; c < ROW_CH; ++c) v[c] += s_prefix[c];
+        for (int j = j0; j < j1; ++j) {
+            const int d = __ldcg(p.deg + r0 + j);
+            store_desc(p.desc, p.desc_off, r0 + j, __ldcg(p.row_start + r0 + j), d, v);
+            row_channels(d, v);
+        }
+        if (slab == S - 1 && tid == 0) {
+            int total[ROW_CH];
+#pragma unroll
+            for (int c = 0; c < ROW_CH; ++c) total[c] = s_prefix[c] + agg[c];
+            write_meta(p.meta, total);
+        }
+        __syncthreads();
+    }
+    if (p.stamp != nullptr && tid == 0) stamp_max(p.stamp + 5, false);
 }
 
 __global__ void compare_csr_kernel(const int *__restrict__ row_start, const int *__restrict__ deg,
@@ -739,36 +848,18 @@
 
 int scan_tiles(int64_t count) { return (int)gp_ceil_div(count > 0 ? count : 1, SCAN_TILE); }
 
-int sort_rows(gp_csr *c, const int *ptr, int *len, int *colbuf, int max_word, bool reset_queue, cudaStream_t stream)
+int sort_rows(gp_csr *c, const int *ptr, int *len, int *colbuf, int max_word, cudaStream_t stream)
 {
     const int64_t n = c->num_nodes;
-    if (reset_queue) GP_LAUNCH(set_meta_kernel, 1, 1, 0, stream, c->meta, GP_META_NUM_BIG_ROWS, 0);
-    GP_LAUNCH_PDL(rowsort_small_kernel, launch_blocks(n, 256), 256, 0, stream, ptr, (const int *)len, colbuf, (long long)n, len,
-                  c->biglist, c->meta, max_word, 1);
-    GP_LAUNCH_PDL(rowsort_big_kernel, gp_sm_count() * 4, BIG_THREADS, (size_t)c->big_smem_bytes, stream, ptr,
-                  (const int *)len, colbuf, len, (const int *)c->biglist, c->meta, max_word, c->bitmap_words,
-                  (const int *)nullptr);
+    GP_LAUNCH(set_meta_kernel, 1, 1, 0, stream, c->meta, GP_META_NUM_BIG_ROWS, 0);
+    GP_LAUNCH(rowsort_small_kernel, launch_blocks(n, 256), 256, 0, stream, ptr, (const int *)len, colbuf, (long long)n, len,
+              c->biglist, c->meta, max_word);
+    GP_LAUNCH(rowsort_big_kernel, gp_sm_count() * 4, BIG_THREADS, (size_t)c->big_smem_bytes, stream, ptr,
+              (const int *)len, colbuf, len, (const int *)c->biglist, c->meta, max_word, c->bitmap_words);
     return GP_OK;
 }
 
-int sort_rows_forked(gp_csr *c, const int *ptr, int *len, int *colbuf, int max_word, cudaStream_t stream)
-{
-    const int64_t n = c->num_nodes;
-    if (c->side == nullptr) {
-        GP_CUDA_CHECK(cudaStreamCreateWithFlags(&c->side, cudaStreamNonBlocking));
-        GP_CUDA_CHECK(cudaEventCreateWithFlags(&c->ev_fork, cudaEventDisableTiming));
-        GP_CUDA_CHECK(cudaEventCreateWithFlags(&c->ev_join, cudaEventDisableTiming));
-    }
-    GP_CUDA_CHECK(cudaEventRecord(c->ev_fork, stream));
-    GP_CUDA_CHECK(cudaStreamWaitEvent(c->side, c->ev_fork, 0));
-    GP_LAUNCH(rowsort_big_kernel, gp_sm_count() * 4, BIG_THREADS, (size_t)c->big_smem_bytes, c->side, ptr, (const int *)len,
-              colbuf, len, (const int *)c->biglist, c->meta, max_word, c->bitmap_words, (const int *)c->medlist);
-    GP_CUDA_CHECK(cudaEventRecord(c->ev_join, c->side));
-    GP_LAUNCH_PDL(rowsort_small_kernel, launch_blocks(n, 256), 256, 0, stream, ptr, (const int *)len, colbuf, (long long)n, len,
-                  c->biglist, c->meta, max_word, 0);
-    GP_CUDA_CHECK(cudaStreamWaitEvent(stream, c->ev_join, 0));
-    return GP_OK;
-}
+size_t build_zero_words(int slabs) { return CB_CTL + (size_t)slabs * (2 + ScanStatus<ROW_CH>::STRIDE); }
 
 }
 
@@ -777,7 +868,9 @@
     GP_REQUIRE(out != nullptr, GP_ERR_INVALID, "gp_csr_create: out is NULL");
     *out = nullptr;
     GP_REQUIRE(num_nodes >= 0 && edge_capacity >= 0, GP_ERR_INVALID, "gp_csr_create: negative size");
-    GP_REQUIRE(num_nodes < (1ll << 31) - 1, GP_ERR_UNSUPPORTED, "gp_csr_create: num_nodes must fit int32");
+    GP_REQUIRE(num_nodes <= (int64_t)CB_MAX_SLABS * CB_MAX_R, GP_ERR_UNSUPPORTED,
+               "gp_csr_create: %lld nodes exceed the %lld (slabs x rows per slab) of this build", (long long)num_nodes,
+               (long long)CB_MAX_SLABS * CB_MAX_R);
     const int64_t kcap = edge_capacity * ((flags & GP_CSR_SYMMETRIZE) ? 2 : 1);
     GP_REQUIRE(kcap < (1ll << 30) - 1, GP_ERR_UNSUPPORTED,
                "gp_csr_create: %lld edge keys exceed the 2^30-1 limit of this build", (long long)kcap);
@@ -825,14 +918,31 @@
     alloc((void **)&c->cursor, (nn + 1) * sizeof(int));
     alloc((void **)&c->col, kc * sizeof(int));
     alloc((void **)&c->biglist, (size_t)c->big_capacity * sizeof(int));
-    c->med_capacity = kcap / 17 + 1;
-    alloc((void **)&c->medlist, (size_t)c->med_capacity * sizeof(int));
     alloc((void **)&c->desc, (size_t)c->desc_capacity * sizeof(int4));
-    c->scan_b_offset = (size_t)scan_tiles(num_nodes + 1) * ScanStatus<1>::STRIDE;
-    c->scan_status_words = c->scan_b_offset + (size_t)scan_tiles(num_nodes + 1) * ScanStatus<ROW_CH>::STRIDE + 8;
-    alloc((void **)&c->meta, (GP_META_WORDS + c->scan_status_words + nn + 1) * sizeof(int));
+    alloc((void **)&c->deg, (nn + 1) * sizeof(int));
+    alloc((void **)&c->bkt_col, kc * sizeof(int));
+    alloc((void **)&c->bkt_row, kc * sizeof(unsigned short));
+    c->slab_off_offset = build_zero_words(CB_MAX_SLABS);
+    c->scan_status_words = std::max(c->slab_off_offset + CB_MAX_SLABS, (size_t)scan_tiles(num_nodes + 1) * ScanStatus<1>::STRIDE) + 8;
+    alloc((void **)&c->meta, (GP_META_WORDS + c->scan_status_words) * sizeof(int));
     c->scan_status = c->meta != nullptr ? c->meta + GP_META_WORDS : nullptr;
-    c->deg = c->meta != nullptr ? c->scan_status + c->scan_status_words : nullptr;
+    if (rc == GP_OK && (cudaMemset(c->meta, 0, (GP_META_WORDS + c->scan_status_words) * sizeof(int)) != cudaSuccess ||
+                        cudaMemset(c->deg, 0, (nn + 1) * sizeof(int)) != cudaSuccess)) {
+        gp_set_error("gp_csr_create: cudaMemset failed");
+        rc = GP_ERR_CUDA;
+    }
+    if (rc == GP_OK) {
+        const int smem = CB_SMEM_INTS * (int)sizeof(int);
+        int occ = 0;
+        if (cudaFuncSetAttribute(csr_build_kernel, cudaFuncAttributeMaxDynamicSharedMemorySize, smem) != cudaSuccess ||
+            cudaOccupancyMaxActiveBlocksPerMultiprocessor(&occ, csr_build_kernel, CB_THREADS, smem) != cudaSuccess ||
+            occ < 1) {
+            cudaGetLastError();
+            gp_set_error("gp_csr_create: csr_build_kernel does not fit on an SM");
+            rc = GP_ERR_CUDA;
+        }
+        c->build_grid = occ * gp_sm_count();
+    }
     if (rc != GP_OK) {
         gp_csr_free(c);
         return rc;
@@ -860,11 +970,6 @@
 {
     if (!c) return GP_OK;
     for (int i = 0; i < 16; ++i) cudaFree(c->scratch[i]);
-    for (int i = 0; i < 12; ++i)
-        if (c->trace_ev[i]) cudaEventDestroy(c->trace_ev[i]);
-    if (c->ev_fork) cudaEventDestroy(c->ev_fork);
-    if (c->ev_join) cudaEventDestroy(c->ev_join);
-    if (c->side) cudaStreamDestroy(c->side);
     cudaFree(c->row_start);
     cudaFree(c->cursor);
     cudaFree(c->col);
@@ -872,8 +977,10 @@
     cudaFree(c->col_in);
     cudaFree(c->deg_in);
     cudaFree(c->biglist);
-    cudaFree(c->medlist);
     cudaFree(c->desc);
+    cudaFree(c->deg);
+    cudaFree(c->bkt_col);
+    cudaFree(c->bkt_row);
     cudaFree(c->meta);
     delete c;
     return GP_OK;
@@ -892,50 +999,49 @@
     c->num_input_edges = num_edges;
     c->built = false;
     c->in_built = false;
-    c->trace_n = 0;
-    auto mark = [&]() {
-        if (!gp_env().csr_trace || c->trace_n >= 12) return;
-        if (c->trace_ev[c->trace_n] == nullptr) cudaEventCreate(&c->trace_ev[c->trace_n]);
-        cudaEventRecordWithFlags(c->trace_ev[c->trace_n++], stream,
-                                 gp_is_capturing() ? cudaEventRecordExternal : cudaEventRecordDefault);
-    };
-    mark();
-    GP_CUDA_CHECK(cudaMemsetAsync(c->meta, 0, (GP_META_WORDS + c->scan_status_words + (size_t)n + 1) * sizeof(int), stream));
-    if (n > 0) {
-        const long long *ei = (const long long *)d_edge_index;
-        const int vec = (reinterpret_cast<uintptr_t>(ei) & 15u) == 0 && num_edges % 2 == 0;
-        int *ticket_a = c->scan_status + c->scan_status_words - 8, *ticket_b = ticket_a + 1;
-        mark();
-        if (num_edges > 0)
-            GP_LAUNCH(count_edges_kernel, launch_blocks(gp_ceil_div(num_edges, 4), 256), 256, 0, stream, ei, num_edges, n, sym,
-                      vec, c->deg, c->meta);
-        mark();
-        PtrScanBuildIo pio{c->deg, c->row_start, c->cursor, n, c->biglist, c->medlist, c->meta};
-        gp_count_launch();
-        GP_CUDA_CHECK(gp_launch_pdl(chained_scan_kernel<1, PtrScanBuildIo, SCAN_IPT>, dim3((unsigned)scan_tiles(n + 1)),
-                                    dim3(SCAN_THREADS), 0, stream, pio, (long long)(n + 1), c->scan_status, ticket_a));
-        mark();
-        if (num_edges > 0)
-            GP_LAUNCH_PDL(scatter_edges_kernel, launch_blocks(gp_ceil_div(num_edges, 4), 256), 256, 0, stream, ei,
-                          (long long)num_edges, (long long)n, sym, vec, c->cursor, c->col);
-        mark();
-        GP_TRY(sort_rows_forked(c, c->row_start, c->deg, c->col, GP_META_MAX_DEGREE, stream));
-        mark();
-        RowScanIo rio;
-        rio.deg = c->deg;
-        rio.row_start = c->row_start;
-        rio.desc = c->desc;
-        for (int k = 0; k < GP_NUM_CLASSES; ++k) rio.off[k] = c->desc_off[k];
-        rio.meta = c->meta;
-        rio.n = n;
-        gp_count_launch();
-        GP_CUDA_CHECK(gp_launch_pdl(chained_scan_kernel<ROW_CH, RowScanIo, SCAN_IPT>, dim3((unsigned)scan_tiles(n)),
-                                    dim3(SCAN_THREADS), 0, stream, rio, (long long)n, c->scan_status + c->scan_b_offset,
-                                    ticket_b));
-        mark();
-        mark();
-    }
-    GP_CUDA_CHECK(cudaGetLastError());
+    if (n == 0) {
+        GP_CUDA_CHECK(cudaMemsetAsync(c->meta, 0, GP_META_WORDS * sizeof(int), stream));
+        c->built = true;
+        return GP_OK;
+    }
+    const int64_t keys = num_edges * (sym ? 2 : 1);
+    int lg = 0;
+    while (((n - 1) >> lg) + 1 > c->build_grid && (1 << lg) < CB_MAX_R) ++lg;
+    while (lg > 0 && (keys << lg) > n * (CB_STAGE / 2)) --lg;
+    while (((n - 1) >> lg) + 1 > CB_MAX_SLABS) ++lg;
+    const int slabs = (int)(((n - 1) >> lg) + 1);
+    GP_CUDA_CHECK(cudaMemsetAsync(c->meta, 0, (GP_META_WORDS + build_zero_words(slabs)) * sizeof(int), stream));
+    c->traced = gp_env().csr_trace != 0;
+    CsrBuildParams p;
+    p.ei = (const long long *)d_edge_index;
+    p.e = num_edges;
+    p.n = n;
+    p.sym = sym;
+    p.vec = (reinterpret_cast<uintptr_t>(d_edge_index) & 15u) == 0 && num_edges % 2 == 0;
+    p.lg = lg;
+    p.slabs = slabs;
+    const int64_t words = (n + 31) / 32;
+    p.bitmap_words = words <= CB_SMEM_INTS ? (int)words : 0;
+    p.chunk = gp_ceil_div(gp_ceil_div(num_edges, c->build_grid), 4) * 4;
+    p.bar = reinterpret_cast<u32 *>(c->scan_status);
+    p.stamp = c->traced ? reinterpret_cast<unsigned long long *>(c->scan_status + 4) : nullptr;
+    p.slab_cnt = c->scan_status + CB_CTL;
+    p.slab_cur = p.slab_cnt + slabs;
+    p.status = p.slab_cur + slabs;
+    p.slab_off = c->scan_status + c->slab_off_offset;
+    p.bkt_col = c->bkt_col;
+    p.bkt_row = c->bkt_row;
+    p.row_start = c->row_start;
+    p.deg = c->deg;
+    p.biglist = c->biglist;
+    p.col = c->col;
+    p.desc = c->desc;
+    for (int k = 0; k < GP_NUM_CLASSES; ++k) p.desc_off[k] = c->desc_off[k];
+    p.meta = c->meta;
+    void *args[] = {&p};
+    gp_count_launch();
+    GP_CUDA_CHECK(cudaLaunchCooperativeKernel((const void *)csr_build_kernel, dim3(c->build_grid), dim3(CB_THREADS), args,
+                                              CB_SMEM_INTS * sizeof(int), stream));
     c->built = true;
     return GP_OK;
 }
@@ -943,10 +1049,13 @@
 extern "C" int gp_csr_trace_ms(gp_csr_t *c, float *ms, int32_t cap, int32_t *num)
 {
     GP_REQUIRE(c != nullptr && ms != nullptr && num != nullptr, GP_ERR_INVALID, "gp_csr_trace_ms: NULL argument");
-    GP_REQUIRE(c->trace_n >= 2, GP_ERR_INVALID, "gp_csr_trace_ms: set GP_CSR_TRACE=1 and build first");
-    GP_CUDA_CHECK(cudaEventSynchronize(c->trace_ev[c->trace_n - 1]));
+    GP_REQUIRE(c->traced && c->num_nodes > 0, GP_ERR_INVALID, "gp_csr_trace_ms: set GP_CSR_TRACE=1 and build first");
+    GP_CUDA_CHECK(cudaDeviceSynchronize());
+    unsigned long long t[6];
+    GP_CUDA_CHECK(cudaMemcpy(t, c->scan_status + 4, sizeof(t), cudaMemcpyDeviceToHost));
+    t[0] = ~t[0];
     int k = 0;
-    for (; k + 1 < c->trace_n && k < cap; ++k) GP_CUDA_CHECK(cudaEventElapsedTime(ms + k, c->trace_ev[k], c->trace_ev[k + 1]));
+    for (; k < 5 && k < cap; ++k) ms[k] = (float)((double)(t[k + 1] - t[k]) * 1e-6);
     *num = k;
     return GP_OK;
 }
@@ -975,7 +1084,7 @@
                                                                                         ticket);
         GP_LAUNCH(scatter_in_kernel, row_blocks(n), 256, 0, stream, c->row_start, c->deg, c->col, n, c->cursor,
                   c->col_in);
-        GP_TRY(sort_rows(c, c->rowptr_in, c->deg_in, c->col_in, GP_META_SCRATCH, true, stream));
+        GP_TRY(sort_rows(c, c->rowptr_in, c->deg_in, c->col_in, GP_META_SCRATCH, stream));
         GP_LAUNCH(compare_csr_kernel, row_blocks(n), 256, 0, stream, c->row_start, c->deg, c->col, c->rowptr_in,
                   c->col_in, n, c->meta);
     }
diff --git a/graphpope_b200/csrc/gp_internal.h b/graphpope_b200/csrc/gp_internal.h
--- a/graphpope_b200/csrc/gp_internal.h
+++ b/graphpope_b200/csrc/gp_internal.h
@@ -18,7 +18,6 @@
     GP_META_IS_SYMMETRIC = 5,
     GP_META_IN_BUILT = 6,
     GP_META_NUM_HUB_ROWS = 7,
-    GP_META_NUM_MED_ROWS = 8,
     GP_META_ENT_BASE = 16,
     GP_META_SLOT_BASE = 24,
     GP_META_WORDS = 32
@@ -46,19 +45,17 @@
     int *col_in = nullptr;
     int *deg_in = nullptr;
     int *biglist = nullptr;
-    int *medlist = nullptr;
-    int64_t med_capacity = 0;
+    int *bkt_col = nullptr;
+    unsigned short *bkt_row = nullptr;
     int4 *desc = nullptr;
     int *meta = nullptr;
     int *scan_status = nullptr;
     size_t scan_status_words = 0;
-    size_t scan_b_offset = 0;
+    size_t slab_off_offset = 0;
+    int build_grid = 0;
     void *scratch[16] = {};
     size_t scratch_bytes[16] = {};
-    cudaStream_t side = nullptr;
-    cudaEvent_t ev_fork = nullptr, ev_join = nullptr;
-    cudaEvent_t trace_ev[12] = {};
-    int trace_n = 0;
+    bool traced = false;
     int bitmap_words = 0;
     int big_smem_bytes = 0;
 };
```

After: 975.1, median of 6. 0.945x the previous value.
